# flynn-nrg/izpi

Hardware: AMD Instinct MI355X
Metric: Msamples/sec (pixels x spp) at 1024x1024/512spp (higher is better)
Workload: dtype f64

## Files before the change

### include/izpi_gpu.h

```cpp
#ifndef IZPI_GPU_H
#define IZPI_GPU_H
#include <stddef.h>
#include <stdint.h>
#include "izpi_types.h"

#ifdef __cplusplus
extern "C" {
#endif

typedef struct izpi_ctx izpi_ctx;

typedef struct izpi_scene_desc {
  uint32_t abi_version;
  uint32_t num_nodes;
  uint32_t num_prims;
  uint32_t num_tris, num_spheres, num_lights, num_materials, num_textures;
  uint32_t num_spd;
  uint32_t flags;
  uint64_t num_texels;
  const izpi_bvh4_node* nodes;
  const uint32_t* prim_ref;
  const double* tri_v0;
  const double* tri_v1;
  const double* tri_v2;
  const double* tri_e1;
  const double* tri_e2;
  const double* tri_normal;
  const double* tri_tangent;
  const double* tri_bitangent;
  const double* tri_uv;
  const double* tri_area;
  const uint32_t* tri_mat;
  const double* sph_center0;
  const double* sph_center1;
  const double* sph_time;
  const double* sph_radius;
  const uint32_t* sph_mat;
  const uint32_t* light_ref;
  const izpi_material* materials;
  const izpi_texture* textures;
  const double* texels;
  const double* spd_wavelengths;
  const double* spd_values;
  izpi_camera camera;
} izpi_scene_desc;

enum {
  IZPI_SCENE_QUANTIZED_BVH = 1
};

enum {
  IZPI_SAMPLER_NORMAL = 1,
  IZPI_SAMPLER_COLOUR = 2,
  IZPI_SAMPLER_WIREFRAME = 3,
  IZPI_SAMPLER_ALBEDO = 4,
  IZPI_SAMPLER_SPECTRAL = 5
};
enum {
  IZPI_OUT_CANVAS = 0,
  IZPI_OUT_PACKED = 1
};

typedef struct izpi_render_tuning {
  uint32_t slots;
  uint32_t chunk_units;
  uint32_t rec_dense;
  uint32_t pool_div;
  uint32_t trace_chunk;
  uint32_t refill_min;
  uint32_t prim_weight;
  uint32_t flags;
  uint64_t tail_paths;
  uint32_t peer_timeout_ms;
  uint32_t pad_tuning;
} izpi_render_tuning;
enum {
  IZPI_TUNE_NO_DIST = 1,
  IZPI_TUNE_GENERAL_TRACE = 2,
  IZPI_TUNE_NO_LEAF_SHORTCUT = 4,
  IZPI_TUNE_SCALAR_SLAB = 8,
  IZPI_TUNE_NO_TAIL = 16,
  IZPI_TUNE_PASS_LOG = 32,
  IZPI_TUNE_NO_LDS_BVH = 64,
  IZPI_TUNE_NO_RAY_LDS = 128,
  IZPI_TUNE_NO_PRIM_LDS = 256,
  IZPI_TUNE_NO_PLACE_PICK = 512,
  IZPI_TUNE_NO_QNODES = 1024,
  IZPI_TUNE_NO_SHADE_STAGE = 2048,
  IZPI_TUNE_WIDE_ADDR = 4096
};

typedef struct izpi_render_req {
  uint32_t width, height;
  uint32_t spp;
  uint32_t max_depth;
  uint32_t sampler;
  uint32_t out_layout;
  uint32_t num_tiles;
  uint32_t num_bg_spd;
  const uint32_t* tiles;
  const double* bg_spd_wavelengths;
  const double* bg_spd_values;
  double background[3];
  uint64_t seed;
  uint32_t post;
  uint32_t abi_version;
  double exposure;
  const izpi_render_tuning* tuning;
  uint32_t accumulation;
  uint32_t pad_req;
  double ink[3];
} izpi_render_req;

enum { IZPI_ACC_RECURSIVE = 0, IZPI_ACC_FORWARD = 1 };

enum { IZPI_POST_NONE = 0, IZPI_POST_SPECTRAL = 1,
       IZPI_POST_GAMMA_CLAMP = 2 };

enum { IZPI_FILTER_GAMMA = 1,
       IZPI_FILTER_CLAMP = 2   };
#define IZPI_MAX_FILTERS 8

typedef struct izpi_render_stats {
  uint64_t rays;
  uint64_t node_visits;
  uint64_t tri_tests;
  uint64_t sph_tests;
  uint64_t light_tri_tests;
  uint64_t light_sph_tests;
  uint64_t samples;
  double kernel_ms;
  double shade_ms;
  double total_ms;
  uint32_t launches;
  uint32_t pad;
  uint64_t node_steps, prim_steps, leaf_shortcuts;
  double tail_ms;
  uint64_t tail_node_visits, tail_tri_tests, tail_sph_tests;
  uint64_t parks;
  uint64_t workspace_bytes, scene_bytes;
  uint32_t slots, rec_dense, pool_blocks, chunk_spp;
  double alloc_ms;
} izpi_render_stats;

typedef struct izpi_hit {
  double t, u, v;
  double p[3];
  double normal[3];
  uint32_t prim_ref;
  uint32_t hit;
} izpi_hit;

int izpi_gpu_open(int device, izpi_ctx** out);
int izpi_gpu_close(izpi_ctx* ctx);
const char* izpi_gpu_last_error(izpi_ctx* ctx);

int izpi_gpu_upload_scene(izpi_ctx* ctx, const izpi_scene_desc* scene);

int izpi_gpu_render(izpi_ctx* ctx, const izpi_render_req* req, double* out_host, izpi_render_stats* stats);

int izpi_gpu_prepare(izpi_ctx* ctx, const izpi_render_req* req);

int izpi_gpu_render_device(izpi_ctx* ctx, const izpi_render_req* req, double* out_dev, izpi_render_stats* stats);

int izpi_gpu_unpack_tiles(izpi_ctx* ctx, const izpi_render_req* req, const double* packed_dev, double* canvas_dev);

int izpi_gpu_spectral_post(izpi_ctx* ctx, const double* xyz_dev, double* rgba_dev, uint32_t width, uint32_t height,
                           double exposure);

int izpi_gpu_postprocess(izpi_ctx* ctx, double* canvas_dev, uint32_t width, uint32_t height, const uint32_t* filters,
                         const double* params, uint32_t num_filters);

typedef struct izpi_denoise_params {
  uint32_t iterations;
  uint32_t flags;
  double sigma_colour, sigma_normal, sigma_albedo;
} izpi_denoise_params;
#define IZPI_DENOISE_MAX_ITERATIONS 8
#define IZPI_DENOISE_DEFAULT_ITERATIONS 5
#define IZPI_DENOISE_DEFAULT_SIGMA_COLOUR 1.0
#define IZPI_DENOISE_DEFAULT_SIGMA_NORMAL 0.5
#define IZPI_DENOISE_DEFAULT_SIGMA_ALBEDO 0.5
int izpi_gpu_denoise_device(izpi_ctx* ctx, const double* colour_dev, const double* normal_dev, const double* albedo_dev,
                            double* out_dev, uint32_t width, uint32_t height, const izpi_denoise_params* p,
                            double* device_ms);
int izpi_gpu_denoise(izpi_ctx* ctx, const double* colour, const double* normal, const double* albedo, double* out,
                     uint32_t width, uint32_t height, const izpi_denoise_params* p, double* device_ms);

enum { IZPI_BVH_LBVH = 0,
       IZPI_BVH_PLOC = 1,
       IZPI_BVH_SAH = 0x100 };
int izpi_gpu_build_bvh4(izpi_ctx* ctx, const double* boxes, uint32_t n, uint32_t leaf_max, uint32_t method,
                        izpi_bvh4_node* nodes, uint32_t max_nodes, uint32_t* num_nodes, uint32_t* order, double* build_ms);

typedef struct izpi_multi izpi_multi;
int izpi_gpu_multi_open(const int* devices, uint32_t num_devices, izpi_multi** out);
int izpi_gpu_multi_close(izpi_multi* m);
const char* izpi_gpu_multi_last_error(izpi_multi* m);
uint32_t izpi_gpu_multi_size(izpi_multi* m);
izpi_ctx* izpi_gpu_multi_context(izpi_multi* m, uint32_t i);
int izpi_gpu_multi_upload_scene(izpi_multi* m, const izpi_scene_desc* scene);
int izpi_gpu_multi_prepare(izpi_multi* m, const izpi_render_req* req);
int izpi_gpu_multi_render(izpi_multi* m, const izpi_render_req* req, double* out_host, izpi_render_stats* stats);

#define IZPI_COMM_ID_BYTES 128
int izpi_gpu_comm_id(uint8_t* id );
int izpi_gpu_comm_init(izpi_ctx* ctx, uint32_t nranks, uint32_t rank, const uint8_t* id );
int izpi_gpu_render_rank(izpi_ctx* ctx, const izpi_render_req* req, double* out_dev, izpi_render_stats* stats);

int izpi_gpu_progress(izpi_ctx* ctx, uint64_t* samples_done, uint64_t* samples_total);
int izpi_gpu_multi_progress(izpi_multi* m, uint64_t* samples_done, uint64_t* samples_total);

enum { IZPI_SNAP_CANVAS = 0, IZPI_SNAP_DISPLAY = 1 };
int izpi_gpu_progressive_begin(izpi_ctx* ctx, const izpi_render_req* req, uint32_t step_spp);
int izpi_gpu_progressive_step(izpi_ctx* ctx, uint32_t spp, izpi_render_stats* stats);
int izpi_gpu_progressive_snapshot(izpi_ctx* ctx, uint32_t form, double* out_host);
int izpi_gpu_progressive_snapshot_device(izpi_ctx* ctx, uint32_t form, double* out_dev);
int izpi_gpu_progressive_end(izpi_ctx* ctx);
int izpi_gpu_multi_progressive_begin(izpi_multi* m, const izpi_render_req* req, uint32_t step_spp);
int izpi_gpu_multi_progressive_step(izpi_multi* m, uint32_t spp, izpi_render_stats* stats);
int izpi_gpu_multi_progressive_snapshot(izpi_multi* m, uint32_t form, double* out_host);
int izpi_gpu_multi_progressive_end(izpi_multi* m);

enum { IZPI_PROG_NOISE = 1 };
enum { IZPI_SNAP_NOISE = 2 };
typedef struct izpi_noise_params {
  double threshold, floor, tolerated;
  uint32_t min_spp;
  uint32_t flags;
} izpi_noise_params;
#define IZPI_NOISE_DEFAULT_THRESHOLD 0.25
#define IZPI_NOISE_DEFAULT_FLOOR 0.01
#define IZPI_NOISE_DEFAULT_TOLERATED 0.05
#define IZPI_NOISE_DEFAULT_MIN_SPP 8
typedef struct izpi_noise_stats {
  uint64_t pixels, nonfinite, above;
  double max_error, sum_error, device_ms;
  uint32_t done, converged;
} izpi_noise_stats;
int izpi_gpu_progressive_begin_ex(izpi_ctx* ctx, const izpi_render_req* req, uint32_t step_spp, uint32_t flags);
int izpi_gpu_progressive_noise(izpi_ctx* ctx, const izpi_noise_params* p, izpi_noise_stats* out);
int izpi_gpu_progressive_converge(izpi_ctx* ctx, const izpi_noise_params* p, izpi_render_stats* stats,
// ... 17 lines not shown
```

### izpi_amd/_native.py

```python
import ctypes as C
from pathlib import Path

ROOT = Path(__file__).resolve().parents[1]
LIB_PATH = ROOT / "izpi_amd" / "_lib" / "libizpi_gpu.so"

c_double_p = C.POINTER(C.c_double)
c_uint32_p = C.POINTER(C.c_uint32)
c_float_p = C.POINTER(C.c_float)

COMM_ID_BYTES = 128
IZPI_OK, IZPI_ERR_INVALID, IZPI_ERR_HIP, IZPI_ERR_NO_SCENE, IZPI_ERR_UNSUPPORTED, IZPI_ERR_DEVICE, IZPI_ERR_PEER = range(7)
IZPI_ABI_VERSION = 4
ACC_RECURSIVE, ACC_FORWARD = 0, 1
SCENE_QUANTIZED_BVH = 1
PRIM_TRIANGLE, PRIM_SPHERE = 0, 1
TEX_CONSTANT, TEX_IMAGE, TEX_SPECTRAL_GAUSSIAN, TEX_SPECTRAL_TABULATED, TEX_SPECTRAL_IMAGE = 1, 3, 5, 7, 9
MAT_DIELECTRIC, MAT_DIFFUSE_LIGHT, MAT_ISOTROPIC, MAT_LAMBERT, MAT_METAL, MAT_PBR = 1, 2, 3, 4, 5, 6
MATF_BEER_LAMBERT = 1
SAMPLER_NORMAL, SAMPLER_COLOUR, SAMPLER_WIREFRAME, SAMPLER_ALBEDO, SAMPLER_SPECTRAL = 1, 2, 3, 4, 5
OUT_CANVAS, OUT_PACKED = 0, 1
POST_NONE, POST_SPECTRAL, POST_GAMMA_CLAMP = 0, 1, 2
SNAP_CANVAS, SNAP_DISPLAY, SNAP_NOISE = 0, 1, 2
PROG_NOISE = 1
NOISE_DEFAULT_THRESHOLD, NOISE_DEFAULT_FLOOR, NOISE_DEFAULT_TOLERATED, NOISE_DEFAULT_MIN_SPP = 0.25, 0.01, 0.05, 8
FILTER_GAMMA, FILTER_CLAMP = 1, 2
MAX_FILTERS = 8
HOST_SKIP_BVH = 1
BVH_LBVH, BVH_PLOC = 0, 1
BVH_SAH = 0x100
BVH_PLOC_SAH = BVH_PLOC | BVH_SAH
DISPLACE_PER_TRIANGLE, DISPLACE_MESH = 0, 1
DISPLACE_MAX_LEVELS = 16
DENOISE_MAX_ITERATIONS = 8
DENOISE_DEFAULT_ITERATIONS = 5
DENOISE_DEFAULT_SIGMA_COLOUR, DENOISE_DEFAULT_SIGMA_NORMAL, DENOISE_DEFAULT_SIGMA_ALBEDO = 1.0, 0.5, 0.5


def prim_ref(kind, idx):
    return (kind << 31) | idx


class BVH4Node(C.Structure):
    _fields_ = [("min_x", C.c_float * 4), ("min_y", C.c_float * 4), ("min_z", C.c_float * 4),
                ("max_x", C.c_float * 4), ("max_y", C.c_float * 4), ("max_z", C.c_float * 4),
                ("child", C.c_int32 * 4), ("prim_count", C.c_int32 * 4)]


class Texture(C.Structure):
    _fields_ = [("kind", C.c_uint32), ("width", C.c_uint32), ("height", C.c_uint32),
                ("spd_offset", C.c_uint32), ("spd_count", C.c_uint32), ("pad0", C.c_uint32),
                ("texel_offset", C.c_uint64), ("value", C.c_double * 3),
                ("peak", C.c_double), ("center", C.c_double), ("width_nm", C.c_double)]


class Material(C.Structure):
    _fields_ = [("kind", C.c_uint32), ("albedo_tex", C.c_int32), ("spectral_tex", C.c_int32),
                ("normal_tex", C.c_int32), ("roughness_tex", C.c_int32), ("metalness_tex", C.c_int32),
                ("absorb_tex", C.c_int32), ("flags", C.c_uint32), ("ref_idx", C.c_double),
                ("fuzz", C.c_double), ("rgb", C.c_double * 3), ("pad1", C.c_double)]


class Camera(C.Structure):
    _fields_ = [("origin", C.c_double * 3), ("lower_left", C.c_double * 3), ("horizontal", C.c_double * 3),
                ("vertical", C.c_double * 3), ("u", C.c_double * 3), ("v", C.c_double * 3),
                ("lens_radius", C.c_double), ("time0", C.c_double), ("time1", C.c_double), ("exposure", C.c_double)]


class SceneDesc(C.Structure):
    _fields_ = [("abi_version", C.c_uint32), ("num_nodes", C.c_uint32), ("num_prims", C.c_uint32),
                ("num_tris", C.c_uint32), ("num_spheres", C.c_uint32), ("num_lights", C.c_uint32),
                ("num_materials", C.c_uint32), ("num_textures", C.c_uint32), ("num_spd", C.c_uint32),
                ("flags", C.c_uint32), ("num_texels", C.c_uint64),
                ("nodes", C.POINTER(BVH4Node)), ("prim_ref", c_uint32_p),
                ("tri_v0", c_double_p), ("tri_v1", c_double_p), ("tri_v2", c_double_p),
                ("tri_e1", c_double_p), ("tri_e2", c_double_p), ("tri_normal", c_double_p),
                ("tri_tangent", c_double_p), ("tri_bitangent", c_double_p), ("tri_uv", c_double_p),
                ("tri_area", c_double_p), ("tri_mat", c_uint32_p),
                ("sph_center0", c_double_p), ("sph_center1", c_double_p), ("sph_time", c_double_p),
                ("sph_radius", c_double_p), ("sph_mat", c_uint32_p),
                ("light_ref", c_uint32_p), ("materials", C.POINTER(Material)), ("textures", C.POINTER(Texture)),
                ("texels", c_double_p), ("spd_wavelengths", c_double_p), ("spd_values", c_double_p),
                ("camera", Camera)]


class RenderTuning(C.Structure):
    _fields_ = [("slots", C.c_uint32), ("chunk_units", C.c_uint32), ("rec_dense", C.c_uint32),
                ("pool_div", C.c_uint32), ("trace_chunk", C.c_uint32), ("refill_min", C.c_uint32),
                ("prim_weight", C.c_uint32), ("flags", C.c_uint32), ("tail_paths", C.c_uint64),
                ("peer_timeout_ms", C.c_uint32), ("pad_tuning", C.c_uint32)]


TUNE_NO_DIST, TUNE_GENERAL_TRACE, TUNE_NO_LEAF_SHORTCUT, TUNE_SCALAR_SLAB, TUNE_NO_TAIL, TUNE_PASS_LOG = 1, 2, 4, 8, 16, 32
TUNE_NO_LDS_BVH = 64
TUNE_NO_RAY_LDS = 128
TUNE_NO_PRIM_LDS = 256
TUNE_NO_QNODES = 1024
TUNE_NO_SHADE_STAGE = 2048
TUNE_WIDE_ADDR = 4096


def tuning(**kw):
    t = RenderTuning()
    for k, v in kw.items():
        if k == "flags" and not isinstance(v, int):
            v = sum(v)
        setattr(t, k, v)
    return t


class RenderReq(C.Structure):
    _fields_ = [("width", C.c_uint32), ("height", C.c_uint32), ("spp", C.c_uint32), ("max_depth", C.c_uint32),
                ("sampler", C.c_uint32), ("out_layout", C.c_uint32), ("num_tiles", C.c_uint32),
                ("num_bg_spd", C.c_uint32), ("tiles", c_uint32_p), ("bg_spd_wavelengths", c_double_p),
                ("bg_spd_values", c_double_p), ("background", C.c_double * 3), ("seed", C.c_uint64),
                ("post", C.c_uint32), ("abi_version", C.c_uint32), ("exposure", C.c_double),
                ("tuning", C.POINTER(RenderTuning)), ("accumulation", C.c_uint32), ("pad_req", C.c_uint32),
                ("ink", C.c_double * 3)]


class RenderStats(C.Structure):
    _fields_ = [("rays", C.c_uint64), ("node_visits", C.c_uint64), ("tri_tests", C.c_uint64),
                ("sph_tests", C.c_uint64), ("light_tri_tests", C.c_uint64), ("light_sph_tests", C.c_uint64),
                ("samples", C.c_uint64), ("kernel_ms", C.c_double), ("shade_ms", C.c_double),
                ("total_ms", C.c_double), ("launches", C.c_uint32), ("pad", C.c_uint32),
                ("node_steps", C.c_uint64), ("prim_steps", C.c_uint64), ("leaf_shortcuts", C.c_uint64),
                ("tail_ms", C.c_double), ("tail_node_visits", C.c_uint64), ("tail_tri_tests", C.c_uint64),
                ("tail_sph_tests", C.c_uint64), ("parks", C.c_uint64), ("workspace_bytes", C.c_uint64),
                ("scene_bytes", C.c_uint64), ("slots", C.c_uint32), ("rec_dense", C.c_uint32),
                ("pool_blocks", C.c_uint32), ("chunk_spp", C.c_uint32), ("alloc_ms", C.c_double)]

    def as_dict(self):
        return {k: getattr(self, k) for k, _ in self._fields_ if k != "pad"}


class DenoiseParams(C.Structure):
    _fields_ = [("iterations", C.c_uint32), ("flags", C.c_uint32), ("sigma_colour", C.c_double),
                ("sigma_normal", C.c_double), ("sigma_albedo", C.c_double)]


def denoise_params(iterations=DENOISE_DEFAULT_ITERATIONS, sigma_colour=DENOISE_DEFAULT_SIGMA_COLOUR,
                   sigma_normal=DENOISE_DEFAULT_SIGMA_NORMAL, sigma_albedo=DENOISE_DEFAULT_SIGMA_ALBEDO):
    return DenoiseParams(int(iterations), 0, float(sigma_colour), float(sigma_normal), float(sigma_albedo))


class NoiseParams(C.Structure):
    _fields_ = [("threshold", C.c_double), ("floor", C.c_double), ("tolerated", C.c_double),
                ("min_spp", C.c_uint32), ("flags", C.c_uint32)]


def noise_params(threshold=NOISE_DEFAULT_THRESHOLD, floor=NOISE_DEFAULT_FLOOR, tolerated=NOISE_DEFAULT_TOLERATED,
                 min_spp=NOISE_DEFAULT_MIN_SPP):
    return NoiseParams(float(threshold), float(floor), float(tolerated), int(min_spp), 0)


class NoiseStats(C.Structure):
    _fields_ = [("pixels", C.c_uint64), ("nonfinite", C.c_uint64), ("above", C.c_uint64),
                ("max_error", C.c_double), ("sum_error", C.c_double), ("device_ms", C.c_double),
                ("done", C.c_uint32), ("converged", C.c_uint32)]

    def as_dict(self):
        return {k: getattr(self, k) for k, _ in self._fields_}


class Hit(C.Structure):
    _fields_ = [("t", C.c_double), ("u", C.c_double), ("v", C.c_double), ("p", C.c_double * 3),
                ("normal", C.c_double * 3), ("prim_ref", C.c_uint32), ("hit", C.c_uint32)]


class TriIn(C.Structure):
    _fields_ = [("v0", C.c_double * 3), ("v1", C.c_double * 3), ("v2", C.c_double * 3),
                ("uv", C.c_double * 6), ("material", C.c_uint32), ("pad", C.c_uint32)]


class SphereIn(C.Structure):
    _fields_ = [("center", C.c_double * 3), ("radius", C.c_double), ("material", C.c_uint32), ("pad", C.c_uint32)]


class CameraIn(C.Structure):
    _fields_ = [("look_from", C.c_double * 3), ("look_at", C.c_double * 3), ("vup", C.c_double * 3),
                ("vfov", C.c_double), ("aspect", C.c_double), ("aperture", C.c_double), ("focus_dist", C.c_double),
                ("time0", C.c_double), ("time1", C.c_double), ("exposure", C.c_double)]


class SceneInput(C.Structure):
    _fields_ = [("num_tris", C.c_uint32), ("num_spheres", C.c_uint32), ("num_materials", C.c_uint32),
                ("num_textures", C.c_uint32), ("num_spd", C.c_uint32), ("pad0", C.c_uint32),
                ("num_texels", C.c_uint64), ("tris", C.c_void_p), ("spheres", C.c_void_p),
                ("materials", C.POINTER(Material)), ("textures", C.POINTER(Texture)), ("texels", c_double_p),
                ("spd_wavelengths", c_double_p), ("spd_values", c_double_p), ("camera", CameraIn),
                ("aspect_override", C.c_double), ("bvh_seed", C.c_uint64)]


COLOUR_RGB, COLOUR_SPECTRAL = 1, 2
OBJ_IGNORE_NORMALS, OBJ_IGNORE_MATERIALS, OBJ_IGNORE_TEXTURES = 1, 2, 4
OBJ_FACE_POLYGON = 1


class ProtoInfo(C.Structure):
    _fields_ = [("colour_representation", C.c_uint32), ("stream_triangles", C.c_uint32),
                ("total_triangles", C.c_uint64), ("num_triangles", C.c_uint32), ("num_streamed_triangles", C.c_uint32),
                ("num_spheres", C.c_uint32), ("num_materials", C.c_uint32), ("num_image_textures", C.c_uint32),
                ("num_displacement_maps", C.c_uint32), ("num_background", C.c_uint32), ("pad", C.c_uint32),
                ("name", C.c_char_p), ("version", C.c_char_p), ("warnings", C.c_char_p)]


class ObjInfo(C.Structure):
    _fields_ = [("has_normals", C.c_uint32), ("has_uv", C.c_uint32), ("ignore_materials", C.c_uint32),
                ("ignore_normals", C.c_uint32), ("ignore_textures", C.c_uint32), ("num_groups", C.c_uint32),
                ("num_materials", C.c_uint32), ("pad", C.c_uint32), ("num_vertices", C.c_uint64),
                ("num_normals", C.c_uint64), ("num_uvs", C.c_uint64), ("centre", C.c_double * 3),
                ("object_name", C.c_char_p)]


class ObjGroup(C.Structure):
    _fields_ = [("name", C.c_char_p), ("material", C.c_char_p), ("face_type", C.c_uint32), ("is_null", C.c_uint32),
                ("num_faces", C.c_uint64), ("num_face_vertices", C.c_uint64)]


class ObjMaterial(C.Structure):
    _fields_ = [("name", C.c_char_p), ("kd", C.c_double * 3), ("ka", C.c_double * 3), ("ks", C.c_double * 3),
                ("num_kd", C.c_uint32), ("num_ka", C.c_uint32), ("num_ks", C.c_uint32), ("pad", C.c_uint32),
                ("ns", C.c_double), ("ni", C.c_double), ("d", C.c_double), ("sharpness", C.c_int64),
                ("illum", C.c_int64)]


ABI_STRUCTS = [BVH4Node, Texture, Material, Camera, SceneDesc, RenderReq, RenderStats, Hit, TriIn, SphereIn, CameraIn,
               SceneInput, ProtoInfo, ObjInfo, ObjGroup, ObjMaterial, RenderTuning, DenoiseParams, NoiseParams, NoiseStats]

EXPORTS = [
    "izpi_gpu_open", "izpi_gpu_close", "izpi_gpu_prepare", "izpi_gpu_multi_prepare", "izpi_gpu_last_error", "izpi_gpu_upload_scene", "izpi_gpu_render",
    "izpi_gpu_render_device", "izpi_gpu_unpack_tiles", "izpi_gpu_output_bytes", "izpi_gpu_trace",
    "izpi_gpu_ray_aabb4", "izpi_gpu_gomath", "izpi_gpu_spectral_post", "izpi_gpu_postprocess",
    "izpi_gpu_build_bvh4", "izpi_gpu_multi_open", "izpi_gpu_multi_close", "izpi_gpu_multi_last_error",
    "izpi_gpu_multi_size", "izpi_gpu_multi_context", "izpi_gpu_multi_upload_scene", "izpi_gpu_multi_render",
    "izpi_gpu_comm_id", "izpi_gpu_comm_init", "izpi_gpu_render_rank", "izpi_gpu_debug_fault", "izpi_gpu_debug_realloc", "izpi_gpu_progress", "izpi_gpu_multi_progress", "izpi_host_build_scene_ex", "izpi_host_scene_prim_boxes", "izpi_host_scene_set_bvh", "izpi_host_scene_set_flags",
    "izpi_host_build_scene", "izpi_host_scene_desc", "izpi_host_scene_stack_bound", "izpi_host_scene_build_ms",
    "izpi_host_scene_free", "izpi_host_last_error", "izpi_host_tiles", "izpi_host_share_units", "izpi_host_share_tiles", "izpi_host_share_block", "izpi_host_assemble_shares", "izpi_host_bvh_leaf_max", "izpi_host_gomath", "izpi_abi_struct_size",
    "izpi_scene_parse_text", "izpi_scene_parse_binary", "izpi_scene_serialize", "izpi_scene_info", "izpi_scene_image_file",
    "izpi_scene_set_image", "izpi_scene_add_triangles", "izpi_scene_background", "izpi_scene_to_input",
    "izpi_scene_material_name", "izpi_scene_free", "izpi_light_source", "izpi_light_source_name",
    "izpi_obj_parse", "izpi_obj_info_get", "izpi_obj_copy_vertices", "izpi_obj_group_get", "izpi_obj_copy_faces",
    "izpi_obj_material_get", "izpi_obj_translate", "izpi_obj_scale", "izpi_obj_rotate",
    "izpi_obj_group_to_triangles", "izpi_obj_free",
    "izpi_gpu_displace", "izpi_host_displace", "izpi_scene_displacement_file", "izpi_scene_set_displacement_map",
    "izpi_scene_set_displacer",
    "izpi_gpu_progressive_begin", "izpi_gpu_progressive_step", "izpi_gpu_progressive_snapshot",
    "izpi_gpu_progressive_snapshot_device", "izpi_gpu_progressive_end",
    "izpi_gpu_multi_progressive_begin", "izpi_gpu_multi_progressive_step", "izpi_gpu_multi_progressive_snapshot",
    "izpi_gpu_multi_progressive_end",
    "izpi_gpu_denoise_device", "izpi_gpu_denoise", "izpi_host_denoise",
    "izpi_gpu_progressive_begin_ex", "izpi_gpu_progressive_noise", "izpi_gpu_progressive_converge",
# ... 144 lines not shown
```

### izpi_amd/csrc/izpi_dev.h

```cpp
#pragma once
#include <hip/hip_runtime.h>
#include <stdint.h>
#include "../../include/izpi_gpu.h"
#include "gomath.h"
#include "scene_records.h"

#define IZPI_DEV __device__ __forceinline__

namespace izd {

struct DevScene {
  const GInner* inner;
  const GInnerQ* innerq;
  const GLeaf* leaves;
  const GPrim* prims;
  const GShade* shade;
  const GTriTex* tritex;
  const GLight* lights;
  const izpi_material* materials;
  const izpi_texture* textures;
  const double4* mat_const;
  const MatTex* mat_tex;
  const double* texels;
  const double* spd_wl;
  const double* spd_val;
  int32_t root;
  uint32_t num_lights;
  uint32_t nan_free_bounds;
  uint32_t leaf_shortcut;
  uint32_t tri_only;
  uint32_t no_pathlen;
  uint32_t num_inner;
  uint32_t num_prims;
  izpi_camera cam;
  uint32_t lds_bytes;
  uint32_t time_free;
  uint32_t quantized;
  uint32_t addr32;
#ifdef IZPI_SHADOW
  const GInner* sh_inner;
  const GLeaf* sh_leaves;
  const GPrim* sh_prims;
#endif
};

struct RenderParams {
  uint32_t width, height, spp, max_depth;
  uint32_t chunk_spp;
  uint32_t s0;
  uint32_t num_pixels;
  uint32_t tile_w, tile_h;
  uint32_t total_units;
  uint32_t lanes;
  uint32_t num_bg_spd;
  const uint32_t* tiles;
  const double* bg_wl;
  const double* bg_val;
  double background[3];
  uint64_t seed;
  double* out;
  double* recs;
  uint32_t* head;
  unsigned long long* counters;
  uint32_t* error;
};

struct Lcg {
  uint32_t s;
  IZPI_DEV double next() {
    s = 1664525u * s + 1013904223u;
    return (double)s / 4294967296.0;
  }
};
IZPI_DEV uint64_t splitmix64(uint64_t x) {
  uint64_t z = x + 0x9E3779B97F4A7C15ull;
  z = (z ^ (z >> 30)) * 0xBF58476D1CE4E5B9ull;
  z = (z ^ (z >> 27)) * 0x94D049BB133111EBull;
  return z ^ (z >> 31);
}
#define IZPI_CAMERA_STREAM_SALT 0xD6E8FEB86659FD93ull

IZPI_DEV int64_t go_int(double x) {
  if (x != x || x >= 9223372036854775808.0 || x < -9223372036854775808.0) return INT64_MIN;
  return (int64_t)x;
}

struct V3 { double x, y, z; };
IZPI_DEV V3 mk(double x, double y, double z) { V3 r; r.x = x; r.y = y; r.z = z; return r; }
IZPI_DEV V3 ld3(const double* p) { return mk(p[0], p[1], p[2]); }
IZPI_DEV V3 add(V3 a, V3 b) { return mk(a.x + b.x, a.y + b.y, a.z + b.z); }
IZPI_DEV V3 sub(V3 a, V3 b) { return mk(a.x - b.x, a.y - b.y, a.z - b.z); }
IZPI_DEV V3 mul(V3 a, V3 b) { return mk(a.x * b.x, a.y * b.y, a.z * b.z); }
IZPI_DEV V3 smul(V3 a, double t) { return mk(a.x * t, a.y * t, a.z * t); }
IZPI_DEV bool sdiv_plain(double x) {
  return ((uint32_t)(__double2hiint(x) >> 20) & 0x7FFu) - (1023u - 300u) <= 600u;
}
IZPI_DEV V3 sdiv(V3 a, double t) {
  const int px = (int)sdiv_plain(a.x) | (int)(a.x == 0.0), py = (int)sdiv_plain(a.y) | (int)(a.y == 0.0),
            pz = (int)sdiv_plain(a.z) | (int)(a.z == 0.0);
  const bool plain = ((int)sdiv_plain(t) & px & py & pz) != 0;
  if (plain) {
    double r = __builtin_amdgcn_rcp(t);
    double e = __builtin_fma(-t, r, 1.0);
    r = __builtin_fma(r, e, r);
    e = __builtin_fma(-t, r, 1.0);
    r = __builtin_fma(r, e, r);
    auto q1 = [&](double n) {
      const double q = n * r;
      const double res = __builtin_fma(-t, q, n);
      return __builtin_amdgcn_div_fixup(__builtin_amdgcn_div_fmas(res, r, q, false), t, n);
    };
    return mk(q1(a.x), q1(a.y), q1(a.z));
  }
  return mk(a.x / t, a.y / t, a.z / t);
}
IZPI_DEV double dot(V3 a, V3 b) { return (a.x * b.x) + (a.y * b.y) + (a.z * b.z); }
IZPI_DEV V3 cross(V3 a, V3 b) { return mk((a.y * b.z) - (a.z * b.y), -((a.x * b.z) - (a.z * b.x)), (a.x * b.y) - (a.y * b.x)); }
IZPI_DEV double sqlen(V3 a) { return (a.x * a.x) + (a.y * a.y) + (a.z * a.z); }
IZPI_DEV double length(V3 a) { return gm::sqrt(sqlen(a)); }
IZPI_DEV V3 unit(V3 a) { return sdiv(a, length(a)); }
IZPI_DEV V3 lerp(V3 a, V3 b, double t) {
  return mk((1 - t) * a.x + t * b.x, (1 - t) * a.y + t * b.y, (1 - t) * a.z + t * b.z);
}
IZPI_DEV bool bad(double x) { return x != x || gm::is_inf(x, 0); }
IZPI_DEV V3 denan(V3 v) { return mk(bad(v.x) ? 0.0 : v.x, bad(v.y) ? 0.0 : v.y, bad(v.z) ? 0.0 : v.z); }

struct Onb {
  V3 u, v, w;
  IZPI_DEV void build(V3 n) {
    w = unit(n);
    V3 a = gm::abs(w.x) > 0.9 ? mk(0, 1, 0) : mk(1, 0, 0);
    v = unit(cross(w, a));
    u = cross(w, v);
  }
  IZPI_DEV V3 local(V3 a) const { return add(add(smul(u, a.x), smul(v, a.y)), smul(w, a.z)); }
};

IZPI_DEV V3 random_cosine_direction(Lcg& r) {
  double r1 = r.next();
  double r2 = r.next();
  double z = gm::sqrt(1 - r2);
  double phi = 6.283185307179586 * r1;
  double sp, cp;
  gm::sincos_nonneg(phi, &sp, &cp);
  double x = cp * 2 * gm::sqrt(r2);
  double y = sp * 2 * gm::sqrt(r2);
  return mk(x, y, z);
}
IZPI_DEV V3 random_to_sphere(double radius, double dist2, Lcg& r) {
  double r1 = r.next();
  double r2 = r.next();
  double z = 1 + r2 * (gm::sqrt(1 - radius * radius / dist2) - 1);
  double phi = 6.283185307179586 * r1;
  double sp, cp;
  gm::sincos_nonneg(phi, &sp, &cp);
  double x = cp * gm::sqrt(1 - z * z);
  double y = sp * gm::sqrt(1 - z * z);
  return mk(x, y, z);
}
IZPI_DEV V3 random_in_unit_sphere(Lcg& r) {
  for (;;) {
    double x = r.next(), y = r.next(), z = r.next();
    V3 p = sub(smul(mk(x, y, z), 2.0), mk(1.0, 1.0, 1.0));
    if (sqlen(p) < 1.0) return p;
  }
}

IZPI_DEV float max32(float a, float b) { return a > b ? a : b; }
IZPI_DEV float min32(float a, float b) { return a < b ? a : b; }
IZPI_DEV bool slab(float mnx, float mny, float mnz, float mxx, float mxy, float mxz, float ox, float oy, float oz,
                   float ix, float iy, float iz, float tmax) {
  float t0x = (mnx - ox) * ix, t1x = (mxx - ox) * ix;
  if (t0x > t1x) { float t = t0x; t0x = t1x; t1x = t; }
  float t0y = (mny - oy) * iy, t1y = (mxy - oy) * iy;
  if (t0y > t1y) { float t = t0y; t0y = t1y; t1y = t; }
  float t0z = (mnz - oz) * iz, t1z = (mxz - oz) * iz;
  if (t0z > t1z) { float t = t0z; t0z = t1z; t1z = t; }
  float tn = max32(max32(t0x, t0y), t0z);
  float tf = min32(min32(t1x, t1y), t1z);
  return tn <= tf && tf >= 0 && tn <= tmax;
}

typedef float f32x2 __attribute__((ext_vector_type(2)));
IZPI_DEV void slab4_fast(float4 mnx, float4 mny, float4 mnz, float4 mxx, float4 mxy, float4 mxz, float ox, float oy,
                         float oz, float ix, float iy, float iz, float tmax, uint64_t (&h)[4]) {
  const f32x2 o_x = {ox, ox}, o_y = {oy, oy}, o_z = {oz, oz};
  const f32x2 i_x = {ix, ix}, i_y = {iy, iy}, i_z = {iz, iz};
  const f32x2 a0x = (f32x2{mnx.x, mnx.y} - o_x) * i_x, a1x = (f32x2{mnx.z, mnx.w} - o_x) * i_x;
  const f32x2 b0x = (f32x2{mxx.x, mxx.y} - o_x) * i_x, b1x = (f32x2{mxx.z, mxx.w} - o_x) * i_x;
  const f32x2 a0y = (f32x2{mny.x, mny.y} - o_y) * i_y, a1y = (f32x2{mny.z, mny.w} - o_y) * i_y;
  const f32x2 b0y = (f32x2{mxy.x, mxy.y} - o_y) * i_y, b1y = (f32x2{mxy.z, mxy.w} - o_y) * i_y;
// ... 87 lines not shown
```

### izpi_amd/csrc/izpi_gpu.hip

```cpp
#include "izpi_kern.h"
#include "noise.h"
#include "scene_pack.h"

#include <array>

using izpi_internal::Double4;
using izpi_internal::pack_scene;
using izpi_internal::PackedScene;
using izpi_internal::trace_addr32;
using izpi_internal::trace_layout;
using izpi_internal::TraceLayout;
using izpi_internal::PlanCache;
using izpi_internal::PlanInput;
using izpi_internal::SideLayout;
using izpi_internal::WorkspacePlan;

__global__ void __launch_bounds__(256) k_spectral_post(const double* in, double* out, uint32_t W, uint32_t H,
                                                       double exposure) {
  __shared__ double ys[18][18];
  const int tx = threadIdx.x & 15, ty = threadIdx.x >> 4;
  const int x0 = blockIdx.x * 16, y0 = blockIdx.y * 16;
  for (int i = threadIdx.x; i < 18 * 18; i += 256) {
    const int hx = x0 + (i % 18) - 1, hy = y0 + (i / 18) - 1;
    ys[i / 18][i % 18] = (hx >= 0 && hx < (int)W && hy >= 0 && hy < (int)H) ? in[((size_t)hy * W + hx) * 4 + 1] : 0.0;
// ... 418 lines not shown

int allocate(izpi_ctx* ctx, const izpi_render_req* req, const RequestShape& rs, const WorkspacePlan& plan, const Tracer& tr,
             const RenderCall& call) {
  const auto bufs = ctx_buffers(ctx);
  const size_t bytes[RENDER_BUFS] = {plan.samples_bytes, plan.recs_bytes, plan.pool_bytes, plan.ring_bytes,
                                     plan.running_bytes, plan.state_bytes, tr.spill_bytes};
  int rc = IZPI_OK;
  if (rs.preview) {
    if ((rc = session_keeps_sums(ctx, call, ctx->running_cap < plan.running_bytes))) return rc;
    for (size_t k = 0; k < RENDER_BUFS && !rc; k++) rc = grow(ctx, bufs[k].p, bufs[k].cap, bytes[k]);
  } else {
    bool fresh = false;
    rc = grow_render_buffers(ctx, bufs.data(), bytes, &fresh);
    if (!rc && (rc = session_keeps_sums(ctx, call, fresh))) return rc;
  }
  if (!rc) rc = grow(ctx, (void**)&ctx->d_tiles, &ctx->tiles_cap, rs.tiles.size() * sizeof(uint32_t));
  if (!rc && !rs.preview) {
    if (req->num_bg_spd && (!req->bg_spd_wavelengths || !req->bg_spd_values)) { ctx->err = "num_bg_spd without the SPD arrays"; return IZPI_ERR_INVALID; }
    rc = grow(ctx, (void**)&ctx->d_bg, &ctx->bg_cap, (2 * (size_t)req->num_bg_spd + 1) * sizeof(double));
  }
  if (!rc) rc = grow(ctx, (void**)&ctx->d_cpart, &ctx->cpart_cap, (size_t)cpart_rows(ctx) * CNT_N * sizeof(unsigned long long));
  if (!rc && !rs.preview && !rs.fwd) rc = grow(ctx, (void**)&ctx->d_finq, &ctx->finq_cap, (size_t)ctx->num_cus * CPART_BLOCKS_PER_CU * FINQ_WORDS * FINQ_CAP * sizeof(unsigned long long));
  if (rc) ctx->plans[rs.preview].valid = false;
  return rc;
}

int touch_workspace(izpi_ctx* ctx, const WorkspacePlan& plan, const RenderCall& call, double alloc_ms) {
  hipStream_t st = ctx->stream;
  HIP_TRY(hipMemsetAsync(ctx->d_state, 0, plan.state_bytes, st));
  HIP_TRY(hipMemsetAsync(ctx->d_samples, 0, plan.samples_bytes, st));
  if (plan.recs_bytes) HIP_TRY(hipMemsetAsync(ctx->d_recs, 0, plan.recs_bytes, st));
  if (call.range.keep) {
    HIP_TRY(hipMemsetAsync(ctx->d_running, 0, plan.running_bytes, st));
    HIP_TRY(hipMemsetAsync(ctx->d_counters, 0, CNT_N * sizeof(unsigned long long), st));
  }
  HIP_TRY(hipStreamSynchronize(st));
  ctx->last = izpi_render_stats{};
  ctx->last.workspace_bytes = workspace_bytes(ctx);
  ctx->last.slots = plan.slots; ctx->last.chunk_spp = plan.chunk; ctx->last.alloc_ms = alloc_ms;
  return IZPI_OK;
}

int begin_frame(izpi_ctx* ctx, const izpi_render_req* req, const RequestShape& rs, const WorkspacePlan& plan, const RenderCall& call,
                size_t nbg) {
  hipStream_t st = ctx->stream;
  HIP_TRY(hipMemcpyAsync(ctx->d_tiles, rs.tiles.data(), rs.tiles.size() * sizeof(uint32_t), hipMemcpyHostToDevice, st));
  if (nbg) {
    HIP_TRY(hipMemcpyAsync(ctx->d_bg, req->bg_spd_wavelengths, nbg * sizeof(double), hipMemcpyHostToDevice, st));
    HIP_TRY(hipMemcpyAsync(ctx->d_bg + nbg, req->bg_spd_values, nbg * sizeof(double), hipMemcpyHostToDevice, st));
  }
  if (!call.range.keep) {
    HIP_TRY(hipMemsetAsync(ctx->d_running, 0, plan.running_bytes, st));
    HIP_TRY(hipMemsetAsync(ctx->d_counters, 0, CNT_N * sizeof(unsigned long long), st));
  }
  HIP_TRY(hipMemsetAsync(ctx->d_cpart, 0, (size_t)cpart_rows(ctx) * CNT_N * sizeof(unsigned long long), st));
  HIP_TRY(hipMemsetAsync(ctx->d_misc, 0, 8 * MISC_STRIDE * sizeof(uint32_t), st));
  return IZPI_OK;
}

ShadeParams shade_params(izpi_ctx* ctx, const izpi_render_req* req, const RequestShape& rs, const WorkspacePlan& plan) {
  ShadeParams sp{};
  sp.width = req->width; sp.height = req->height; sp.tile_w = rs.tw; sp.tile_h = rs.th; sp.slots = plan.slots;
  sp.max_depth = rs.preview ? 1 : req->max_depth;
  sp.tiles = ctx->d_tiles; sp.seed = req->seed; sp.out = ctx->d_samples;
  sp.background[0] = req->background[0]; sp.background[1] = req->background[1]; sp.background[2] = req->background[2];
  sp.counters = ctx->d_counters; sp.cpart = ctx->d_cpart; sp.error = misc(ctx, 1);
  return sp;
}
void path_shade_params(izpi_ctx* ctx, const izpi_render_req* req, const DevScene& sc, const RequestShape& rs,
                       const WorkspacePlan& plan, size_t nbg, ShadeParams& sp) {
  sp.num_bg_spd = (uint32_t)nbg;
  sp.bg_sorted = nbg >= 2;
  for (size_t i = 1; i < nbg; i++)
    if (!(req->bg_spd_wavelengths[i - 1] <= req->bg_spd_wavelengths[i])) sp.bg_sorted = 0;
  sp.bg_wl = ctx->d_bg; sp.bg_val = ctx->d_bg + nbg;
  sp.rec_dense = plan.rec_dense; sp.rec_pool = plan.rec_pool; sp.pool_shift = plan.pool_shift;
  sp.recs = rs.fwd ? nullptr : ctx->d_recs; sp.mat_const = sc.mat_const; sp.head = misc(ctx, 0);
  sp.num_mc = ctx->num_materials; sp.num_tex = ctx->num_textures; sp.num_spd = ctx->num_spd;
  sp.pool = plan.rec_pool ? ctx->d_pool : nullptr; sp.pool_ring = plan.rec_pool ? ctx->d_ring : nullptr;
  sp.pool_ctr = plan.rec_pool ? ctx->d_pool_ctr : nullptr;
  sp.finq = ctx->d_finq;
}
void stage_tables(const izpi_ctx* ctx, const izpi_render_req* req, const izpi_render_tuning& tu, const RequestShape& rs,
                  const WorkspacePlan& plan, size_t nbg, DevScene& sc, ShadeParams& sp) {
  sp.staged = ctx->num_materials <= MC_LDS && ctx->num_materials <= MAT_LDS && sc.num_lights <= LT_LDS &&
              ctx->num_textures <= TEX_LDS && ctx->num_spd <= SPD_LDS && nbg <= BG_LDS;
  sp.prims_staged = sc.num_prims <= PR_LDS && !(tu.flags & IZPI_TUNE_NO_PRIM_LDS);
  if (sp.staged && (req->sampler == IZPI_SAMPLER_SPECTRAL || ctx->num_spd)) sp.staged = 2;
  if (rs.fwd && req->sampler == IZPI_SAMPLER_COLOUR && ctx->matset == 0 && sp.staged == 1 && !plan.rec_pool && !plan.time &&
      !plan.cold && !(tu.flags & IZPI_TUNE_NO_SHADE_STAGE))
    sp.prims_staged = 0;
  sc.lds_bytes = sp.prims_staged ? lds_off::END : sp.staged == 2 ? lds_off::SPECTRAL_END : sp.staged ? lds_off::COLOUR_END : 0;
  if (tu.flags & IZPI_TUNE_PASS_LOG)
    fprintf(stderr, "IZPI_SHADE_TABLES tables=%u prims=%u lds_bytes=%u\n", sp.staged, sp.prims_staged, sc.lds_bytes);
}
WaveParams wave_params(izpi_ctx* ctx, const WorkspacePlan& plan, const ShadeParams& sp) {
  WaveParams wp{};
  wp.in = bind_side(ctx->d_state, plan, plan.side[0]); wp.out = bind_side(ctx->d_state, plan, plan.side[1]);
  wp.trace_next = misc(ctx, 2); wp.slots = plan.slots;
  wp.read_kind = !ctx->sc.no_pathlen ? 1u : 0u;
  wp.hit_uv = plan.uv ? 1u : 0u;
  wp.pool_ctr = sp.pool_ctr;
  wp.cpart = ctx->d_cpart;
  return wp;
}
PreviewParams preview_params(izpi_ctx* ctx, const izpi_render_req* req, const WorkspacePlan& plan) {
  PreviewParams pp{};
  pp.buf = bind_side(ctx->d_state, plan, plan.side[0]);
  pp.tminmax = plan.tminmax ? (double2*)(ctx->d_state + plan.side[0].tminmax) : nullptr;
  pp.slots = plan.slots;
  pp.verts = ctx->d_triverts;
  if (req->abi_version >= 4)
    for (int k = 0; k < 3; k++) pp.ink[k] = req->ink[k];
  return pp;
}
AccumParams accum_params(izpi_ctx* ctx, const izpi_render_req* req, const RequestShape& rs, double* out_dev) {
  AccumParams ap{};
  ap.num_pixels = rs.num_pixels; ap.spp = req->spp; ap.width = req->width; ap.height = req->height;
  ap.tile_w = rs.tw; ap.tile_h = rs.th; ap.out_layout = req->out_layout;
  ap.sampler = rs.preview ? (uint32_t)IZPI_SAMPLER_COLOUR : req->sampler;
  ap.tiles = ctx->d_tiles; ap.samples = ctx->d_samples; ap.running = ctx->d_running; ap.out = out_dev;
  return ap;
}

int guard_status(izpi_ctx* ctx, uint32_t guard) {
  if (!guard) return IZPI_OK;
  ctx->err = guard & 1u   ? "device guard: traversal stack overflow"
             : guard & 2u ? "device guard: unknown material kind"
                            : "device guard: no overflow record block in k_tail";
  return IZPI_ERR_DEVICE;
}

int render_body(izpi_ctx* ctx, const izpi_render_req* req, const RenderCall& call, double* out_dev) {
  const auto t_body0 = std::chrono::steady_clock::now();
  auto host_ms = [&t_body0]() { return std::chrono::duration<double, std::milli>(std::chrono::steady_clock::now() - t_body0).count(); };
  RequestShape rs;
  int rc = check_request(ctx, req, &rs);
  if (rc) return rc;
  const SampleRange& sr = call.range;
  const uint32_t num_pixels = rs.num_pixels;
  if (sr.keep) {
    izpi_ctx::Session& ss = ctx->session;
    ss.run_tiles = rs.tiles; ss.tile_w = rs.tw; ss.tile_h = rs.th; ss.num_pixels = num_pixels;
  }
  const izpi_render_tuning& tu = tuning_of(req);
  const bool pass_log = (tu.flags & IZPI_TUNE_PASS_LOG) != 0;
  DevScene sc = ctx->sc;
  if (tu.flags & IZPI_TUNE_NO_LEAF_SHORTCUT) sc.leaf_shortcut = 0;
  if (tu.flags & IZPI_TUNE_SCALAR_SLAB) sc.nan_free_bounds = 0;
  Tracer tr;
  const double t_tiles = host_ms();
  if ((rc = make_tracer(ctx, tu, !ctx->sc.tri_only || ctx->any_uv, &tr))) return rc;
  if (pass_log)
    fprintf(stderr, "IZPI_TRACE_INSTANCE dist=%d tri=%d lds_bvh=%d ray_lds=%d q=%d\nIZPI_TRACE_ADDR a32=%d ring=%d\n", (int)tr.p2, (int)tr.tri,
            (int)tr.lds_bvh, (int)tr.ray_lds, (int)tr.qnodes, (int)(tr.a32 && !tr.lds_bvh), trace_ring(tr));
  const double t_tracer = host_ms();
  PlanCache& cache = ctx->plans[rs.preview];
  PlanInput in = plan_input(ctx, req, rs, tu, call.size_spp);
  const bool reuse = cache.find(in) != nullptr;
  if (!reuse) in.avail = available_bytes(ctx);
  const double t_meminfo = host_ms();
  if (!reuse) cache.store(in, plan_workspace(in));
  const WorkspacePlan& plan = cache.plan;
  const double t_sized = host_ms();
  const auto t_alloc0 = std::chrono::steady_clock::now();
  if ((rc = allocate(ctx, req, rs, plan, tr, call))) return rc;
  const double alloc_ms = std::chrono::duration<double, std::milli>(std::chrono::steady_clock::now() - t_alloc0).count();
  if (call.prepare_only) return touch_workspace(ctx, plan, call, alloc_ms);
  hipStream_t st = ctx->stream;
  if (pass_log) HIP_TRY(hipEventRecord(ctx->evb[0], st));
  const size_t nbg = rs.preview ? 0 : req->num_bg_spd;
  if ((rc = begin_frame(ctx, req, rs, plan, call, nbg))) return rc;
  ShadeParams sp = shade_params(ctx, req, rs, plan);
  AccumParams ap = accum_params(ctx, req, rs, out_dev);
  if (!rs.preview) {
    path_shade_params(ctx, req, sc, rs, plan, nbg, sp);
    stage_tables(ctx, req, tu, rs, plan, nbg, sc, sp);
  }

  const RunInput run{num_pixels, plan.chunk, plan.pool_blocks, sr};
  RunTimes times;
  float total_ms = 0;
  const double t_launch = host_ms();
  HIP_TRY(hipEventRecord(ctx->ev0, st));
  if (pass_log) {
    HIP_TRY(hipEventSynchronize(ctx->ev0));
    float prep = 0;
    HIP_TRY(hipEventElapsedTime(&prep, ctx->evb[0], ctx->ev0));
    fprintf(stderr, "IZPI_T ev0_synced %.3f prep_gpu_ms %.3f body_start %.3f\n", diag_clock_ms(), prep,
            diag_clock_ms() - host_ms());
  }
  if (rs.preview) {
    const PreviewParams pp = preview_params(ctx, req, plan);
    rc = run_preview(ctx, req, sc, tr, sp, pp, ap, run, &times);
  } else {
    WaveParams wp = wave_params(ctx, plan, sp);
    const ShadeKernels* k = ctx->kernels[req->sampler == IZPI_SAMPLER_SPECTRAL][rs.fwd];
    if (!k || (!rs.fwd && k->rec_doubles != plan.D)) {
      ctx->err = "the shading instance and the workspace plan disagree on the record stride";
      return IZPI_ERR_INVALID;
    }
    rc = run_wavefront(ctx, req, sc, tr, *k, sp, wp, ap, run, &times);
  }
  if (rc) return rc;
  hipLaunchKernelGGL(k_cpart_reduce, dim3(CNT_N), dim3(256), 0, st, ctx->d_cpart, cpart_rows(ctx), ctx->d_counters);
  HIP_TRY(hipGetLastError());
  HIP_TRY(hipEventRecord(ctx->ev1, st));
  if (!sr.keep && (rc = apply_post(ctx, req, out_dev))) return rc;
  const double t_issued = host_ms();
  HIP_TRY(hipEventSynchronize(ctx->ev1));
  if (pass_log)
    fprintf(stderr, "IZPI_HOST tiles %.3f tracer %.3f meminfo %.3f sized %.3f allocated %.3f launched %.3f issued %.3f done %.3f ms\n",
            t_tiles, t_tracer, t_meminfo, t_sized, t_sized + alloc_ms, t_launch, t_issued, host_ms());
  HIP_TRY(hipEventElapsedTime(&total_ms, ctx->ev0, ctx->ev1));
  unsigned long long cnt[CNT_N];
  uint32_t guard = 0;
  HIP_TRY(hipMemcpy(cnt, ctx->d_counters, sizeof(cnt), hipMemcpyDeviceToHost));
  HIP_TRY(hipMemcpy(&guard, misc(ctx, 1), sizeof(guard), hipMemcpyDeviceToHost));
  izpi_render_stats& s = ctx->last;
  memset(&s, 0, sizeof(s));
  s.rays = cnt[CNT_RAYS]; s.node_visits = cnt[CNT_NODES]; s.tri_tests = cnt[CNT_TRI]; s.sph_tests = cnt[CNT_SPH];
  s.light_tri_tests = cnt[CNT_LTRI]; s.light_sph_tests = cnt[CNT_LSPH];
  s.samples = (uint64_t)num_pixels * sr.end;
  s.kernel_ms = times.trace_ms; s.shade_ms = times.shade_ms; s.total_ms = total_ms; s.launches = times.launches; s.tail_ms = times.tail_ms;
  s.node_steps = cnt[CNT_NSTEP]; s.prim_steps = cnt[CNT_PSTEP]; s.leaf_shortcuts = cnt[CNT_SHORT];
  s.tail_node_visits = cnt[CNT_TAIL_NODES]; s.tail_tri_tests = cnt[CNT_TAIL_TRI]; s.tail_sph_tests = cnt[CNT_TAIL_SPH];
  s.parks = cnt[CNT_PARK];
  s.workspace_bytes = workspace_bytes(ctx);
  s.scene_bytes = ctx->scene_bytes;
  s.slots = plan.slots; s.rec_dense = rs.fwd ? 0 : plan.rec_dense; s.pool_blocks = plan.pool_blocks; s.chunk_spp = plan.chunk;
  s.alloc_ms = alloc_ms;
  if (!sr.keep && plan.rec_pool && s.parks * 64 > s.rays && plan.pool_blocks < plan.slots) ctx->pool_grow++;
#ifdef IZPI_SHADE_CLOCKS
  fprintf(stderr, "IZPI_SHADE_CLOCKS item %llu refill %llu push %llu mat %llu finish %llu mix %llu lpdf %llu entry %llu tex %llu "
          "res_barrier1 %llu res_atomics %llu res_barrier2 %llu (wave cycles; res_atomics: thread 0 only)\n",
          cnt[CNT_SCLK_ITEM], cnt[CNT_SCLK_REFILL], cnt[CNT_SCLK_PUSH], cnt[CNT_SCLK_MAT], cnt[CNT_SCLK_FIN],
          cnt[CNT_SCLK_MIX], cnt[CNT_SCLK_LPDF], cnt[CNT_SCLK_ENTRY], cnt[CNT_SCLK_TEX], cnt[CNT_SCLK_RB1],
          cnt[CNT_SCLK_RATOM], cnt[CNT_SCLK_RB2]);
#endif
#ifdef IZPI_SHADOW
  fprintf(stderr, "IZPI_SHADOW spill_stores %llu spill_loads %llu (entries)\n", cnt[CNT_CLK_REFILL], cnt[CNT_CLK_NODE]);
#endif
#ifdef IZPI_TRACE_ICOUNT
  fprintf(stderr, "IZPI_TRACE_ICOUNT {\"iterations\": %llu, \"idle\": %llu, \"dequeue\": %llu, \"refill\": %llu, \"prim\": %llu, \"node_fast\": %llu, "
          "\"node_twin\": %llu, \"spill\": %llu, \"readback\": %llu, \"pop\": %llu, \"finish\": %llu, \"waves\": %llu}\n",
          cnt[CNT_IC_ITER], cnt[CNT_IC_IDLE], cnt[CNT_IC_DEQUEUE], cnt[CNT_IC_REFILL], cnt[CNT_PSTEP], cnt[CNT_NSTEP] - cnt[CNT_IC_TWIN], cnt[CNT_IC_TWIN],
          cnt[CNT_IC_SPILL], cnt[CNT_IC_READBACK], cnt[CNT_IC_POP], cnt[CNT_IC_FINISH], cnt[CNT_IC_WAVES]);
#endif
#ifdef IZPI_TRACE_CLOCKS
  fprintf(stderr, "IZPI_TRACE_CLOCKS refill %llu node %llu prim %llu advance %llu (wave cycles)\n", cnt[CNT_CLK_REFILL],
          cnt[CNT_CLK_NODE], cnt[CNT_CLK_PRIM], cnt[CNT_CLK_ADV]);
#endif
  return guard_status(ctx, guard);
}

int render_impl(izpi_ctx* ctx, const izpi_render_req* req, const RenderCall& call, double* out_dev) {
  if (session_open(ctx)) return IZPI_ERR_INVALID;
  ctx->prog_done.store(0, std::memory_order_relaxed);
  ctx->prog_total.store(0, std::memory_order_relaxed);
  const int rc = render_body(ctx, req, call, out_dev);
  ctx->prog_done.store(ctx->prog_total.load(std::memory_order_relaxed), std::memory_order_relaxed);
  return rc;
}

struct Shares {
  std::vector<uint32_t> all;
  uint32_t n = 1;
  uint32_t tw = 0, th = 0;
  size_t block = 0;
  std::vector<uint32_t> mine(uint32_t r) const {
    std::vector<uint32_t> t(all.size());
    t.resize(4 * (size_t)izpi_host_share_tiles(all.data(), (uint32_t)(all.size() / 4), r, n, t.data()));
    return t;
  }
};

size_t share_block(size_t ntiles, uint32_t tw, uint32_t th, uint32_t n) { return ((ntiles + n - 1) / n) * (size_t)tw * th * 4; }

int make_shares(izpi_ctx* ctx, const izpi_render_req* req, uint32_t n, Shares& sh) {
  if (!req || req->width == 0 || req->height == 0) { ctx->err = "invalid render request"; return IZPI_ERR_INVALID; }
  if (req->out_layout != IZPI_OUT_CANVAS) { ctx->err = "multi-GPU renders produce a canvas (IZPI_OUT_CANVAS)"; return IZPI_ERR_INVALID; }
  std::vector<uint32_t> tiles;
  int rc = request_tiles(ctx, req, tiles);
  if (rc) return rc;
  sh.all.resize(4 * tiles.size());
  sh.all.resize(4 * (size_t)izpi_host_share_units(tiles.data(), (uint32_t)(tiles.size() / 4), n, sh.all.data()));
  if (!validate_tiles(req, sh.all.data(), (uint32_t)(sh.all.size() / 4), &sh.tw, &sh.th)) {
    ctx->err = "tiles must be non-empty, in bounds and equal-sized";
    return IZPI_ERR_INVALID;
  }
  sh.n = n;
  sh.block = share_block(sh.all.size() / 4, sh.tw, sh.th, n);
  return IZPI_OK;
}

int share_buffers(izpi_ctx* ctx, const Shares& sh, bool root, size_t canvas_bytes = 0) {
  int rc = grow(ctx, (void**)&ctx->d_share, &ctx->share_cap, sh.block * sizeof(double));
  if (!rc && root) rc = grow(ctx, (void**)&ctx->d_gather, &ctx->gather_cap, (size_t)sh.n * sh.block * sizeof(double));
  if (!rc && root && canvas_bytes) rc = grow(ctx, (void**)&ctx->d_out, &ctx->out_cap, canvas_bytes);
  return rc;
}

int render_share(izpi_ctx* ctx, const izpi_render_req* req, const Shares& sh, uint32_t r, bool prepare_only = false) {
  const std::vector<uint32_t> mine = sh.mine(r);
  memset(&ctx->last, 0, sizeof(ctx->last));
  if (mine.empty()) return IZPI_OK;
  izpi_render_req q = request_copy(req);
  q.num_tiles = (uint32_t)(mine.size() / 4);
  q.tiles = mine.data();
  q.out_layout = IZPI_OUT_PACKED;
  q.post = IZPI_POST_NONE;
  return render_impl(ctx, &q, one_shot(&q, prepare_only), prepare_only ? nullptr : ctx->d_share);
}

int assemble(izpi_ctx* ctx, const izpi_render_req* req, const Shares& sh, double* canvas_dev) {
  izpi_ctx* root = ctx;
  hipStream_t st = root->stream;
  for (uint32_t r = 0; r < sh.n; r++) {
    const std::vector<uint32_t> t = sh.mine(r);
    if (t.empty()) continue;
    int rc = grow(root, (void**)&root->d_utiles, &root->utiles_cap, sh.all.size() * sizeof(uint32_t));
    if (rc) return rc;
    HIP_TRY(hipMemcpyAsync(root->d_utiles, t.data(), t.size() * sizeof(uint32_t), hipMemcpyHostToDevice, st));
    const uint32_t np = (uint32_t)(t.size() / 4) * sh.tw * sh.th;
    hipLaunchKernelGGL(k_unpack, dim3((np + 255) / 256), dim3(256), 0, st, root->d_utiles, np, sh.tw, sh.th, req->width,
                       req->height, root->d_gather + (size_t)r * sh.block, canvas_dev);
    HIP_TRY(hipGetLastError());
    HIP_TRY(hipStreamSynchronize(st));
  }
  int rc = apply_post(root, req, canvas_dev);
  if (rc) return rc;
  HIP_TRY(hipStreamSynchronize(st));
  return IZPI_OK;
}

int session_copy_request(izpi_ctx::Session& ss, const izpi_render_req* req, std::string& err) {
  ss = izpi_ctx::Session{};
  ss.req = request_copy(req);
  ss.tuning = tuning_of(req);
  ss.req.tuning = req->tuning ? &ss.tuning : nullptr;
  if (ss.req.num_tiles) {
    if (!ss.req.tiles) { err = "num_tiles without tiles"; return IZPI_ERR_INVALID; }
    ss.tiles.assign(ss.req.tiles, ss.req.tiles + 4 * (size_t)ss.req.num_tiles);
    ss.req.tiles = ss.tiles.data();
  }
  if (ss.req.num_bg_spd) {
    if (!ss.req.bg_spd_wavelengths || !ss.req.bg_spd_values) { err = "num_bg_spd without the SPD arrays"; return IZPI_ERR_INVALID; }
    ss.bg_wl.assign(ss.req.bg_spd_wavelengths, ss.req.bg_spd_wavelengths + ss.req.num_bg_spd);
    ss.bg_val.assign(ss.req.bg_spd_values, ss.req.bg_spd_values + ss.req.num_bg_spd);
    ss.req.bg_spd_wavelengths = ss.bg_wl.data();
    ss.req.bg_spd_values = ss.bg_val.data();
  }
  return IZPI_OK;
}

void session_drop(izpi_ctx* ctx) {
  ctx->session = izpi_ctx::Session{};
  ctx->prog_done.store(0, std::memory_order_relaxed);
  ctx->prog_total.store(0, std::memory_order_relaxed);
}

int session_zero_moments(izpi_ctx* ctx) {
  izpi_ctx::Session& ss = ctx->session;
  const size_t bytes = (size_t)ss.num_pixels * 3 * sizeof(double);
  const int rc = grow(ctx, (void**)&ctx->d_moments, &ctx->moments_cap, bytes);
  if (rc) return rc;
  HIP_TRY(hipMemsetAsync(ctx->d_moments, 0, bytes, ctx->stream));
  HIP_TRY(hipStreamSynchronize(ctx->stream));
  ss.noise = true;
  return IZPI_OK;
}

int session_begin(izpi_ctx* ctx, const izpi_render_req* req, uint32_t step_spp, uint32_t flags = 0) {
  if (ctx->session.open) { ctx->err = "a progressive session is already open"; return IZPI_ERR_INVALID; }
  if (!req || step_spp == 0) { ctx->err = "progressive_begin: a request and step_spp >= 1"; return IZPI_ERR_INVALID; }
  if (flags & ~(uint32_t)IZPI_PROG_NOISE) { ctx->err = "progressive_begin: unknown flags"; return IZPI_ERR_INVALID; }
  izpi_ctx::Session& ss = ctx->session;
  int rc = session_copy_request(ss, req, ctx->err);
  if (!rc) {
    ss.step_spp = std::min(step_spp, std::max(1u, ss.req.spp));
    rc = render_body(ctx, &ss.req, RenderCall{SampleRange{0, 0, true}, ss.step_spp, true}, nullptr);
  }
  if (!rc && (flags & IZPI_PROG_NOISE)) rc = session_zero_moments(ctx);
  if (rc) {
    const std::string why = ctx->err;
    session_drop(ctx);
    ctx->err = why;
    return rc;
  }
  ss.cum = izpi_render_stats{};
  ss.open = true;
  ctx->prog_done.store(0, std::memory_order_relaxed);
  ctx->prog_total.store((uint64_t)ss.num_pixels * ss.req.spp, std::memory_order_relaxed);
  return IZPI_OK;
}

int session_usable(izpi_ctx* ctx) {
  if (!ctx->session.open) { ctx->err = "no progressive session is open"; return IZPI_ERR_INVALID; }
  if (ctx->session.broken) { ctx->err = "the session's last step failed: end it"; return IZPI_ERR_INVALID; }
  return IZPI_OK;
// ... 86 lines not shown
  return IZPI_OK;
}

template <class Step, class Noise, class Done>
int converge_loop(const izpi_noise_params* params, uint32_t cap, Step step, Noise noise, Done done, izpi_noise_stats* out) {
  const izpi_noise_params p = params ? *params : nz::defaults();
  izpi_noise_stats last{};
  int rc = IZPI_OK;
  while (!rc && done() < cap) {
    if ((rc = step())) break;
    if (done() < std::max(2u, p.min_spp)) continue;
    if ((rc = noise(&p, &last))) break;
    if (last.converged) break;
  }
  if (out) *out = last;
  return rc;
}

int session_snapshot(izpi_ctx* ctx, uint32_t form, double* out_dev) {
  int rc = session_usable(ctx);
  if (rc) return rc;
  const izpi_ctx::Session& ss = ctx->session;
  if (form != IZPI_SNAP_CANVAS && form != IZPI_SNAP_DISPLAY && form != IZPI_SNAP_NOISE) { ctx->err = "unknown snapshot form"; return IZPI_ERR_INVALID; }
  if (ss.done == 0) { ctx->err = "snapshot before the session's first sample"; return IZPI_ERR_INVALID; }
  if (form == IZPI_SNAP_NOISE && (rc = session_has_noise(ctx))) return rc;
  if (!out_dev) { ctx->err = "null output"; return IZPI_ERR_INVALID; }
  hipStream_t st = ctx->stream;
  if ((rc = session_tiles(ctx))) return rc;
  if (form == IZPI_SNAP_NOISE) {
    NoiseParams np = noise_params(ctx);
    np.out = out_dev;
    launch_noise_resolve(st, np);
    HIP_TRY(hipGetLastError());
    HIP_TRY(hipStreamSynchronize(st));
    return IZPI_OK;
  }
  ResolveParams rp{};
  rp.num_pixels = ss.num_pixels; rp.done = ss.done; rp.width = ss.req.width; rp.height = ss.req.height;
  rp.tile_w = ss.tile_w; rp.tile_h = ss.tile_h; rp.sampler = ss.req.sampler; rp.out_layout = ss.req.out_layout;
  rp.form = form; rp.exposure = ss.req.exposure;
  rp.tiles = ctx->d_tiles; rp.running = ctx->d_running; rp.out = out_dev;
  launch_resolve(st, rp);
  HIP_TRY(hipGetLastError());
  if (form == IZPI_SNAP_CANVAS && (rc = apply_post(ctx, &ss.req, out_dev))) return rc;
  HIP_TRY(hipStreamSynchronize(st));
  return IZPI_OK;
}

}

struct izpi_multi {
  std::vector<izpi_ctx*> ctx;
  std::string err;
  bool prog_open = false;
  izpi_ctx::Session session;
  Shares shares;
};

namespace {
int multi_shares(izpi_multi* m, const izpi_render_req* req, Shares& sh) {
  izpi_ctx* root = m->ctx[0];
  int rc = make_shares(root, req, (uint32_t)m->ctx.size(), sh);
  if (!rc && hipSetDevice(root->device) != hipSuccess) { root->err = "hipSetDevice"; rc = IZPI_ERR_HIP; }
  if (!rc) rc = share_buffers(root, sh, true, (size_t)req->width * req->height * 4 * sizeof(double));
  if (rc) m->err = root->err;
  return rc;
}

template <class F>
int on_every_device(izpi_multi* m, F fn) {
  const uint32_t G = (uint32_t)m->ctx.size();
  std::vector<int> rcs(G, IZPI_OK);
  std::vector<std::thread> th;
  for (uint32_t i = 0; i < G; i++) {
    th.emplace_back([&, i]() {
      izpi_ctx* c = m->ctx[i];
      if (hipSetDevice(c->device) != hipSuccess) { c->err = "hipSetDevice"; rcs[i] = IZPI_ERR_HIP; return; }
      rcs[i] = fn(i, c);
    });
  }
  for (std::thread& t : th) t.join();
  for (uint32_t i = 0; i < G; i++)
    if (rcs[i]) { m->err = "device " + std::to_string(i) + ": " + m->ctx[i]->err; return rcs[i]; }
  return IZPI_OK;
}

bool multi_lacks_noise(izpi_multi* m) {
  if (!m->session.noise) { m->err = "noise: the session was begun without IZPI_PROG_NOISE"; return true; }
  if (m->session.done < 2) { m->err = "noise: needs at least 2 samples"; return true; }
  return false;
}

bool multi_session_open(izpi_multi* m) {
  if (!m->prog_open) return false;
  m->err = "a progressive session is open";
  return true;
}

static_assert(sizeof(Double4) == sizeof(double4), "PackedScene::mat_const uploads as DevScene::mat_const");

int begin_upload(izpi_ctx* ctx, const izpi_scene_desc* d) {
  if (!ctx || !d) return IZPI_ERR_INVALID;
  if (d->abi_version < 1 || d->abi_version > IZPI_ABI_VERSION) { ctx->err = "ABI version mismatch"; return IZPI_ERR_INVALID; }
  if (session_open(ctx)) return IZPI_ERR_INVALID;
  HIP_TRY(hipSetDevice(ctx->device));
  HIP_TRY(hipStreamSynchronize(ctx->stream));
  free_scene(ctx);
  return IZPI_OK;
}

int upload_packed(izpi_ctx* ctx, const izpi_scene_desc* d, const PackedScene& ps) {
  DevScene& sc = ctx->sc;
  memset(&sc, 0, sizeof(sc));
  GInner* di; GInnerQ* dq; GLeaf* dl; GPrim* dp; GShade* dsh; GTriVerts* dtv; GTriTex* dtt; GLight* dlt;
  izpi_material* dm; Double4* dmc; MatTex* dmt; izpi_texture* dtx;
  double *dtex, *dswl, *dsv;
  {
    const TraceLayout tl = trace_layout(ps.inner.size(), ps.innerq.size(), ps.leaves.size());
    char* nb;
    UP((const char*)nullptr, tl.bytes, &nb);
    di = reinterpret_cast<GInner*>(nb);
    dq = ps.innerq.empty() ? nullptr : reinterpret_cast<GInnerQ*>(nb + tl.innerq_at);
    dl = reinterpret_cast<GLeaf*>(nb + tl.leaves_at);
    HIP_TRY(hipMemcpy(di, ps.inner.data(), ps.inner.size() * sizeof(GInner), hipMemcpyHostToDevice));
    if (dq) HIP_TRY(hipMemcpy(dq, ps.innerq.data(), ps.innerq.size() * sizeof(GInnerQ), hipMemcpyHostToDevice));
    HIP_TRY(hipMemcpy(dl, ps.leaves.data(), ps.leaves.size() * sizeof(GLeaf), hipMemcpyHostToDevice));
  }
  UP(ps.prims.data(), ps.prims.size(), &dp);
  UP(ps.shade.data(), ps.shade.size(), &dsh);
  UP(ps.triverts.data(), ps.triverts.size(), &dtv);
  UP(ps.tritex.data(), ps.tritex.size(), &dtt);
  UP(ps.lights.data(), ps.lights.size(), &dlt);
  UP(d->materials, d->num_materials, &dm);
  UP(ps.mat_const.data(), ps.mat_const.size(), &dmc);
  UP(ps.mat_tex.data(), ps.mat_tex.size(), &dmt);
  UP(ps.textures.data(), ps.textures.size(), &dtx);
  UP(ps.texels.data(), ps.texels.size(), &dtex);
  UP(d->spd_wavelengths, d->num_spd, &dswl);
  UP(d->spd_values, d->num_spd, &dsv);
#ifdef IZPI_SHADOW
  {
    GInner* si; GLeaf* sl; GPrim* sp;
    UP(ps.inner.data(), ps.inner.size(), &si);
    UP(ps.leaves.data(), ps.leaves.size(), &sl);
    UP(ps.prims.data(), ps.prims.size(), &sp);
    sc.sh_inner = si; sc.sh_leaves = sl; sc.sh_prims = sp;
  }
#endif
  sc.inner = di; sc.innerq = dq; sc.leaves = dl; sc.prims = dp; sc.shade = dsh; sc.tritex = dtt; sc.lights = dlt;
  sc.materials = dm; sc.mat_const = (const double4*)dmc; sc.mat_tex = dmt; sc.textures = dtx; sc.texels = dtex;
  sc.spd_wl = dswl; sc.spd_val = dsv;
  sc.root = ps.root; sc.num_inner = ps.num_inner; sc.num_prims = d->num_prims; sc.num_lights = d->num_lights;
  sc.quantized = ps.quantized; sc.leaf_shortcut = ps.leaf_shortcut; sc.nan_free_bounds = ps.nan_free_bounds;
  sc.tri_only = ps.tri_only; sc.time_free = ps.time_free; sc.no_pathlen = ps.no_pathlen;
  sc.addr32 = trace_addr32(ps.inner.size(), ps.innerq.size(), ps.leaves.size(), ps.prims.size());
  sc.cam = d->camera;
  ctx->d_triverts = dtv;
  ctx->mat_ok_rgb = ps.mat_ok_rgb; ctx->mat_ok_spectral = ps.mat_ok_spectral;
  ctx->basic_materials = ps.basic_materials; ctx->matset = ps.matset;
  ctx->const_albedo = ps.const_albedo; ctx->any_uv = ps.any_uv;
  ctx->pool_grow = 0;
  ctx->stack_needed = ps.stack_needed;
  ctx->num_prims = d->num_prims;
  ctx->num_textures = d->num_textures;
  ctx->num_materials = d->num_materials;
  ctx->num_spd = d->num_spd;
  ctx->have_scene = true;
  ctx->plans[0].valid = ctx->plans[1].valid = false;
  Tracer tr;
  int rc = make_tracer(ctx, kDefaultTuning, !ctx->sc.tri_only || ctx->any_uv, &tr);
  const bool const_basic = ctx->basic_materials && ctx->const_albedo;
  for (int s = 0; s < 2; s++)
    for (int f = 1; f >= 0; f--) {
      const uint32_t sampler = s ? IZPI_SAMPLER_SPECTRAL : IZPI_SAMPLER_COLOUR;
      const ShadeKernels*& k = ctx->kernels[s][f];
      k = (s ? ctx->mat_ok_spectral : ctx->mat_ok_rgb) ? shade_instance(ctx->matset, const_basic, sampler, f != 0) : nullptr;
      if (!rc && k) rc = prepare_wavefront(ctx, *k);
    }
  if (!rc) rc = prepare_preview(ctx);
  return rc;
}
}

extern "C" {

int izpi_gpu_open(int device, izpi_ctx** out) {
  if (!out) return IZPI_ERR_INVALID;
  *out = nullptr;
  int n = 0;
  hipError_t e = hipGetDeviceCount(&n);
  if (e != hipSuccess || n == 0 || device < 0 || device >= n) return IZPI_ERR_HIP;
  if (hipSetDevice(device) != hipSuccess) return IZPI_ERR_HIP;
  izpi_ctx* ctx = new izpi_ctx();
  ctx->device = device;
  hipDeviceProp_t prop;
  bool ok = hipGetDeviceProperties(&prop, device) == hipSuccess;
  ctx->num_cus = ok ? prop.multiProcessorCount : 0;
  ok = ok && hipStreamCreateWithFlags(&ctx->stream, hipStreamNonBlocking) == hipSuccess &&
       hipEventCreate(&ctx->ev0) == hipSuccess && hipEventCreate(&ctx->ev1) == hipSuccess &&
       hipEventCreate(&ctx->ev2) == hipSuccess && hipEventCreate(&ctx->ev3) == hipSuccess &&
       hipHostMalloc((void**)&ctx->h_count, 9 * MISC_STRIDE * sizeof(uint32_t), hipHostMallocDefault) == hipSuccess &&
       hipMalloc((void**)&ctx->d_misc, 8 * MISC_STRIDE * sizeof(uint32_t)) == hipSuccess &&
       hipMalloc((void**)&ctx->d_pool_ctr, POOL_SHARDS * POOL_CTR_STRIDE * sizeof(unsigned long long)) == hipSuccess &&
       hipMalloc((void**)&ctx->d_counters, CNT_N * sizeof(unsigned long long)) == hipSuccess;
  for (int i = 0; ok && i < 3 * IZPI_PASS_BATCH; i++) ok = hipEventCreate(&ctx->evb[i]) == hipSuccess;
  if (!ok) {
    izpi_gpu_close(ctx);
    return IZPI_ERR_HIP;
  }
  *out = ctx;
  return IZPI_OK;
}

int izpi_gpu_close(izpi_ctx* ctx) {
  if (!ctx) return IZPI_OK;
  (void)hipSetDevice(ctx->device);
  if (ctx->stream) (void)hipStreamSynchronize(ctx->stream);
  if (ctx->comm) (void)ncclCommDestroy(ctx->comm);
  free_scene(ctx);
  for (const CtxBuf& b : ctx_buffers(ctx)) if (*b.p) (void)hipFree(*b.p);
  void* fixed[] = {ctx->d_pool_ctr, ctx->d_misc, ctx->d_counters, ctx->d_status};
  for (void* p : fixed) if (p) (void)hipFree(p);
  if (ctx->h_count) (void)hipHostFree(ctx->h_count);
  if (ctx->stall_host) (void)hipHostFree(ctx->stall_host);
  for (int i = 0; i < 3 * IZPI_PASS_BATCH; i++) if (ctx->evb[i]) (void)hipEventDestroy(ctx->evb[i]);
  hipEvent_t evs[] = {ctx->ev0, ctx->ev1, ctx->ev2, ctx->ev3};
  for (hipEvent_t ev : evs) if (ev) (void)hipEventDestroy(ev);
  if (ctx->stream) (void)hipStreamDestroy(ctx->stream);
  delete ctx;
  return IZPI_OK;
}

const char* izpi_gpu_last_error(izpi_ctx* ctx) { return ctx ? ctx->err.c_str() : "null context"; }

int izpi_gpu_upload_scene(izpi_ctx* ctx, const izpi_scene_desc* d) {
  int rc = begin_upload(ctx, d);
  if (rc) return rc;
  PackedScene ps;
  rc = pack_scene(d, &ps, &ctx->err);
  return rc ? rc : upload_packed(ctx, d, ps);
}

uint64_t izpi_gpu_output_bytes(const izpi_render_req* req) {
  if (!req) return 0;
  if (req->out_layout == IZPI_OUT_PACKED && req->num_tiles) {
    uint64_t px = 0;
    for (uint32_t i = 0; i < req->num_tiles; i++) {
      const uint32_t* t = req->tiles + 4 * i;
      px += (uint64_t)(t[2] - t[0] + 1) * (t[3] - t[1] + 1);
    }
    return px * 4 * sizeof(double);
  }
  return (uint64_t)req->width * req->height * 4 * sizeof(double);
}

int izpi_gpu_render_device(izpi_ctx* ctx, const izpi_render_req* req, double* out_dev, izpi_render_stats* stats) {
  if (!ctx) return IZPI_ERR_INVALID;
  if (!out_dev) { ctx->err = "null output"; return IZPI_ERR_INVALID; }
  HIP_TRY(hipSetDevice(ctx->device));
  int rc = render_impl(ctx, req, one_shot(req), out_dev);
  if (stats) *stats = ctx->last;
  return rc;
}

int izpi_gpu_render(izpi_ctx* ctx, const izpi_render_req* req, double* out_host, izpi_render_stats* stats) {
  if (!ctx) return IZPI_ERR_INVALID;
  if (!out_host || !req) { ctx->err = "null argument"; return IZPI_ERR_INVALID; }
  if (session_open(ctx)) return IZPI_ERR_INVALID;
  HIP_TRY(hipSetDevice(ctx->device));
  const size_t bytes = izpi_gpu_output_bytes(req);
  int rc = grow(ctx, (void**)&ctx->d_out, &ctx->out_cap, bytes);
  if (rc) return rc;
  HIP_TRY(hipMemcpyAsync(ctx->d_out, out_host, bytes, hipMemcpyHostToDevice, ctx->stream));
  rc = render_impl(ctx, req, one_shot(req), ctx->d_out);
  if (stats) *stats = ctx->last;
  if (rc) return rc;
  HIP_TRY(hipMemcpyAsync(out_host, ctx->d_out, bytes, hipMemcpyDeviceToHost, ctx->stream));
  HIP_TRY(hipStreamSynchronize(ctx->stream));
  return IZPI_OK;
}

int izpi_gpu_prepare(izpi_ctx* ctx, const izpi_render_req* req) {
  if (!ctx) return IZPI_ERR_INVALID;
  if (!req) { ctx->err = "null argument"; return IZPI_ERR_INVALID; }
  if (session_open(ctx)) return IZPI_ERR_INVALID;
  HIP_TRY(hipSetDevice(ctx->device));
  if (ctx->comm && ctx->comm_size > 1) {
    Shares sh;
    int rc = make_shares(ctx, req, ctx->comm_size, sh);
    if (!rc) rc = share_buffers(ctx, sh, ctx->comm_rank == 0);
    return rc ? rc : render_share(ctx, req, sh, ctx->comm_rank, true);
  }
  return render_impl(ctx, req, one_shot(req, true), nullptr);
}

int izpi_gpu_progressive_begin_ex(izpi_ctx* ctx, const izpi_render_req* req, uint32_t step_spp, uint32_t flags) {
  if (!ctx) return IZPI_ERR_INVALID;
  HIP_TRY(hipSetDevice(ctx->device));
  return session_begin(ctx, req, step_spp, flags);
}

int izpi_gpu_progressive_begin(izpi_ctx* ctx, const izpi_render_req* req, uint32_t step_spp) {
  return izpi_gpu_progressive_begin_ex(ctx, req, step_spp, 0);
}

int izpi_gpu_progressive_noise(izpi_ctx* ctx, const izpi_noise_params* p, izpi_noise_stats* out) {
  if (!ctx) return IZPI_ERR_INVALID;
// ... 708 lines not shown
```

### izpi_amd/csrc/izpi_kern.h

```cpp
#pragma once
#include <hip/hip_runtime.h>
#include <stdio.h>
#include <stdlib.h>
#include <string.h>
#include <algorithm>
#include <cmath>
#include <string>
#include <vector>

#include <rccl/rccl.h>

#include <atomic>
#include <chrono>
#include <thread>

#include "../../include/izpi_host.h"
#include "../../include/izpi_gpu_debug.h"
#include "izpi_dev.h"
#include "izpi_req.h"
#include "render_plan.h"
#include "cie_tables.h"

using namespace izd;

#define HIP_TRY(expr)                                                                  \
  do {                                                                                 \
    hipError_t e_ = (expr);                                                            \
    if (e_ != hipSuccess) {                                                            \
      ctx->err = std::string(#expr) + ": " + hipGetErrorString(e_);                    \
      return IZPI_ERR_HIP;                                                             \
    }                                                                                  \
  } while (0)

static __constant__ double c_cie_wl[IZPI_CIE_N] = IZPI_CIE_WAVELENGTHS_INIT;
static __constant__ double c_cie_x[IZPI_CIE_N] = IZPI_CIE_X_INIT;
static __constant__ double c_cie_y[IZPI_CIE_N] = IZPI_CIE_Y_INIT;
static __constant__ double c_cie_z[IZPI_CIE_N] = IZPI_CIE_Z_INIT;
struct CieCum { double v[IZPI_CIE_N]; };
constexpr CieCum cie_y_running_sums() {
  CieCum c{};
  constexpr double y[IZPI_CIE_N] = IZPI_CIE_Y_INIT;
  double cur = 0.0;
  for (int i = 0; i < IZPI_CIE_N; i++) { c.v[i] = cur + y[i]; cur += y[i]; }
  return c;
}
static __constant__ CieCum c_cie_ycum = cie_y_running_sums();

namespace izpi_bvh {
int build(hipStream_t st, const double* h_boxes, uint32_t n, uint32_t leaf_max, uint32_t method,
          std::vector<izpi_bvh4_node>& nodes, std::vector<uint32_t>& order, float* ms, std::string& err);
}

#define IZPI_PASS_BATCH 8
constexpr uint32_t SHADE_THREADS = 256, SHADE_WAVES = SHADE_THREADS / 64;
constexpr uint32_t FINQ_WORDS = 5, FINQ_FLUSH = 1024, FINQ_CAP = FINQ_FLUSH + SHADE_THREADS;
constexpr int MISC_STRIDE = 64;

enum { CNT_RAYS = 0, CNT_NODES, CNT_TRI, CNT_SPH, CNT_LTRI, CNT_LSPH, CNT_NSTEP, CNT_PSTEP, CNT_SHORT,
       CNT_CLK_REFILL, CNT_CLK_NODE, CNT_CLK_PRIM, CNT_CLK_ADV, CNT_TAIL_NODES, CNT_TAIL_TRI, CNT_TAIL_SPH,
       CNT_SCLK_ITEM, CNT_SCLK_REFILL, CNT_SCLK_PUSH, CNT_PARK, CNT_SCLK_MAT, CNT_SCLK_FIN, CNT_SCLK_MIX, CNT_SCLK_LPDF,
       CNT_SCLK_ENTRY, CNT_SCLK_TEX, CNT_SCLK_RB1, CNT_SCLK_RATOM, CNT_SCLK_RB2,
       CNT_N };
#ifdef IZPI_TRACE_ICOUNT
enum { CNT_IC_ITER = CNT_CLK_REFILL, CNT_IC_DEQUEUE = CNT_CLK_NODE, CNT_IC_REFILL = CNT_CLK_PRIM, CNT_IC_TWIN = CNT_CLK_ADV,
       CNT_IC_SPILL = CNT_SCLK_ITEM, CNT_IC_READBACK = CNT_SCLK_REFILL, CNT_IC_POP = CNT_SCLK_PUSH, CNT_IC_FINISH = CNT_SCLK_MAT,
       CNT_IC_WAVES = CNT_SCLK_FIN, CNT_IC_IDLE = CNT_SCLK_MIX };
#if defined(IZPI_TRACE_CLOCKS) || defined(IZPI_SHADE_CLOCKS) || defined(IZPI_SHADOW)
#error "IZPI_TRACE_ICOUNT shares counter rows with the clock and shadow builds"
#endif
#endif

IZPI_DEV void count_add(unsigned long long* cpart, unsigned long long* counters, int k, unsigned long long v) {
  if (v == 0) return;
  if (cpart) cpart[(size_t)__builtin_amdgcn_readfirstlane(blockIdx.x * (blockDim.x >> 6) + (threadIdx.x >> 6)) * CNT_N + k] += v;
  else atomicAdd(counters + k, v);
}

template <class T>
IZPI_DEV T sld(const T* p) { return *p; }
template <class T>
IZPI_DEV void sst(T* p, const T& v) { *p = v; }

template <class T>
IZPI_DEV T lds_ld(const T* p) {
  if constexpr (sizeof(T) % 8 == 0 && alignof(T) >= 8) {
    T r;
    uint64_t* d = reinterpret_cast<uint64_t*>(&r);
    const __attribute__((address_space(3))) uint64_t* q = (const __attribute__((address_space(3))) uint64_t*)p;
#pragma unroll
    for (uint32_t i = 0; i < sizeof(T) / 8; i++) d[i] = q[i];
    return r;
  } else {
    return *(const __attribute__((address_space(3))) T*)p;
  }
}

template <bool L, class T>
IZPI_DEV T tld(const T* p) {
  if constexpr (L) return lds_ld(p);
  else return *p;
}
constexpr uint32_t MAT_LDS = 64, TEX_LDS = 64, SPD_LDS = 384, BG_LDS = 128, MT_LDS = 64, LT_LDS = 64, PR_LDS = 64;
namespace lds_off {
constexpr uint32_t al(uint64_t b) { return (uint32_t)((b + 31) & ~31ull); }
constexpr uint32_t MC = 0;
constexpr uint32_t MT = MC + al(MT_LDS * sizeof(double4));
constexpr uint32_t LT = MT + al(MT_LDS * sizeof(MatTex));
constexpr uint32_t LT2 = LT + al(LT_LDS * 16 * sizeof(double));
constexpr uint32_t MAT = LT2 + al(LT_LDS * 6 * sizeof(double));
constexpr uint32_t TEX = MAT + al(MAT_LDS * sizeof(izpi_material));
constexpr uint32_t COLOUR_END = TEX + al(TEX_LDS * sizeof(izpi_texture));
constexpr uint32_t SPD = COLOUR_END;
constexpr uint32_t SPDV = SPD + al(SPD_LDS * sizeof(double));
constexpr uint32_t CIE = SPDV + al(SPD_LDS * sizeof(double));
constexpr uint32_t BG = CIE + al(5 * IZPI_CIE_N * sizeof(double));
constexpr uint32_t BGV = BG + al(BG_LDS * sizeof(double));
constexpr uint32_t SPECTRAL_END = BGV + al(BG_LDS * sizeof(double));
constexpr uint32_t GS = SPECTRAL_END;
constexpr uint32_t TT = GS + al(PR_LDS * sizeof(GShade));
constexpr uint32_t GP = TT + al(PR_LDS * sizeof(GTriTex));
constexpr uint32_t END = GP + al(PR_LDS * sizeof(GPrim));
constexpr uint32_t STG_RAY = COLOUR_END;
constexpr uint32_t STG_THR = STG_RAY + 3 * SHADE_THREADS * 16;
constexpr uint32_t STG_PATH = STG_THR + 3 * SHADE_THREADS * 8;
constexpr uint32_t STG_KIND = STG_PATH + SHADE_THREADS * 16;
constexpr uint32_t STG_END = STG_KIND + SHADE_THREADS * 4;
constexpr uint32_t STG_BYTES = STG_END - COLOUR_END;
}
IZPI_DEV char* lds_arena() {
  extern __shared__ __attribute__((aligned(16))) char izpi_lds_arena[];
  return izpi_lds_arena;
}
IZPI_DEV izpi_material* mat_lds() { return (izpi_material*)(lds_arena() + lds_off::MAT); }
IZPI_DEV izpi_texture* tex_lds() { return (izpi_texture*)(lds_arena() + lds_off::TEX); }
IZPI_DEV double* spd_lds() { return (double*)(lds_arena() + lds_off::SPD); }
IZPI_DEV double* spdv_lds() { return (double*)(lds_arena() + lds_off::SPDV); }
IZPI_DEV double* cie_lds() { return (double*)(lds_arena() + lds_off::CIE); }
IZPI_DEV double* bg_lds() { return (double*)(lds_arena() + lds_off::BG); }
IZPI_DEV double* bgv_lds() { return (double*)(lds_arena() + lds_off::BGV); }
IZPI_DEV izpi_material mat_rec(const DevScene& sc, bool st, uint32_t m) {
  if (st) return lds_ld(mat_lds() + m);
  return sc.materials[m];
}
IZPI_DEV izpi_texture tex_rec(const DevScene& sc, bool st, int32_t id) {
  if (st) return lds_ld(tex_lds() + id);
  return sc.textures[id];
}

IZPI_DEV V3 image_rgb(const double* texels, uint64_t off, uint32_t w, uint32_t h, uint32_t fmt, double u, double v) {
  int64_t i = go_int(u * (double)w);
  int64_t j = go_int((1 - v) * ((double)h - 0.001));
  if (i < 0) i = 0;
  if (j < 0) j = 0;
  if (i > (int64_t)w - 1) i = (int64_t)w - 1;
  if (j > (int64_t)h - 1) j = (int64_t)h - 1;
  uint64_t k = (uint64_t)j * w + (uint64_t)i;
  if (fmt == TEXF_GRAY) {
    const double g = texels[off + k];
    return mk(g, g, g);
  }
  const double* px = texels + off + k * 4;
  const double2 rg = *reinterpret_cast<const double2*>(px);
  return mk(rg.x, rg.y, px[2]);
}
IZPI_DEV uint64_t image_index(uint32_t w, uint32_t h, double u, double v) {
  int64_t i = go_int(u * (double)w);
  int64_t j = go_int((1 - v) * ((double)h - 0.001));
  if (i < 0) i = 0;
  if (j < 0) j = 0;
  if (i > (int64_t)w - 1) i = (int64_t)w - 1;
  if (j > (int64_t)h - 1) j = (int64_t)h - 1;
  return (uint64_t)j * w + (uint64_t)i;
}
IZPI_DEV V3 image_at(const double* texels, uint64_t off, uint32_t fmt, uint64_t k) {
  if (fmt == TEXF_GRAY) {
    const double g = texels[off + k];
    return mk(g, g, g);
  }
  const double* px = texels + off + k * 4;
  const double2 rg = *reinterpret_cast<const double2*>(px);
  return mk(rg.x, rg.y, px[2]);
}
IZPI_DEV V3 tex_rgb(const DevScene& sc, int32_t id, double u, double v, bool st = false) {
  const izpi_texture t = tex_rec(sc, st, id);
  if (t.kind == IZPI_TEX_IMAGE) return image_rgb(sc.texels, t.texel_offset, t.width, t.height, t.pad0, u, v);
  return mk(t.value[0], t.value[1], t.value[2]);
}
IZPI_DEV V3 slot_rgb(const DevScene& sc, const TexSlot& s, double u, double v, bool st = false) {
  const uint32_t fmt = s.hf >> 30;
  if (fmt <= TEXF_GRAY) return image_rgb(sc.texels, s.off, s.w, s.hf & 0x3FFFFFFFu, fmt, u, v);
  return tex_rgb(sc, (int32_t)s.off, u, v, st);
}
IZPI_DEV bool slot_set(const TexSlot& s) { return (s.hf >> 30) != TEXF_NONE; }
IZPI_DEV V3 slot_rgb_k(const DevScene& sc, const TexSlot& s, double u, double v, bool st, uint32_t w0, uint32_t h0, uint64_t k0) {
  const uint32_t fmt = s.hf >> 30, h = s.hf & 0x3FFFFFFFu;
  if (fmt <= TEXF_GRAY) {
    uint64_t k = k0;
    if (s.w != w0 || h != h0) k = image_index(s.w, h, u, v);
    return image_at(sc.texels, s.off, fmt, k);
  }
  return slot_rgb(sc, s, u, v, st);
}
IZPI_DEV MatTex* mt_lds() { return (MatTex*)(lds_arena() + lds_off::MT); }
IZPI_DEV TexSlot mat_slot(const DevScene& sc, bool staged, uint32_t m, int k) {
  if (staged) return lds_ld(&mt_lds()[m].s[k]);
  return sc.mat_tex[m].s[k];
}
template <bool L = false>
IZPI_DEV uint32_t sorted_interval(const double* wl, uint32_t n, double w) {
  uint32_t lo = 1, hi = n - 1;
  while (lo < hi) {
    const uint32_t mid = (lo + hi) >> 1;
    if (tld<L>(wl + mid) >= w) hi = mid; else lo = mid + 1;
  }
  return lo - 1;
}

IZPI_DEV double spectral_image_value(double r, double g, double b, double wl) {
  double sv = 0;
// ... 964 lines not shown
  Shade shade, shade_staged;
  Tail tail32, tail64;
  Shade start;
  void (*refill)(DevScene, ShadeParams, WaveParams, const uint32_t*);
  uint32_t sampler, rec_doubles;
  int matset;
  bool fwd;
  char name[24];
};
template <int SAMPLER, bool FWD>
const ShadeKernels* shade_kernels(int matset);

struct SampleRange {
  uint32_t begin, end;
  bool keep;
};
struct ResolveParams {
  uint32_t num_pixels, done, width, height, tile_w, tile_h, sampler, out_layout;
  uint32_t form;
  double exposure;
  const uint32_t* tiles;
  const double* running;
  double* out;
};
void launch_resolve(hipStream_t st, const ResolveParams& rp);
struct NoiseParams {
  uint32_t num_pixels, done, width, height, tile_w, tile_h, sampler, out_layout;
  double threshold, floor;
  const uint32_t* tiles;
  const double* running;
  const double* moments;
  double* out;
  double* block_sums;
  unsigned long long* block_counts;
};
void launch_noise_resolve(hipStream_t st, const NoiseParams& np);
void launch_noise_stats(hipStream_t st, const NoiseParams& np);
static_assert(sizeof(RayOD) == izpi_internal::plan_size::RAY && sizeof(PathHot) == izpi_internal::plan_size::PATH_HOT &&
                  sizeof(PathCold) == izpi_internal::plan_size::PATH_COLD && sizeof(double2) == izpi_internal::plan_size::HIT,
              "render_plan.h: entry records");
static_assert(SMP_D == izpi_internal::plan_size::SMP_D && POOL_SHARDS == izpi_internal::plan_size::POOL_SHARDS,
              "render_plan.h: per-sample results, pool rings");
static_assert(RecLayout<IZPI_SAMPLER_COLOUR, MATSET_FULL>::D == izpi_internal::plan_size::REC_COLOUR &&
                  RecLayout<IZPI_SAMPLER_COLOUR, MATSET_CONST>::D == izpi_internal::plan_size::REC_COMPACT &&
                  RecLayout<IZPI_SAMPLER_SPECTRAL, MATSET_FULL>::D == izpi_internal::plan_size::REC_SPECTRAL,
              "render_plan.h: record strides");
struct DevBufs {
  std::vector<void*> p;
  template <typename T>
  hipError_t alloc(T** out, size_t count) {
    *out = nullptr;
    const hipError_t e = hipMalloc((void**)out, count * sizeof(T));
    if (e == hipSuccess) p.push_back(*out);
    return e;
  }
  ~DevBufs() {
    for (void* q : p) (void)hipFree(q);
  }
};

struct izpi_ctx {
  int device = 0;
  std::string err;
  hipStream_t stream = nullptr;
  hipEvent_t ev0 = nullptr, ev1 = nullptr, ev2 = nullptr;
  int num_cus = 0;
  bool have_scene = false;
  uint32_t num_textures = 0;
  uint32_t num_materials = 0;
  uint32_t num_spd = 0;
  izpi_internal::PlanCache plans[2];
  const GTriVerts* d_triverts = nullptr;
  DevScene sc{};
  uint32_t stack_needed = 0;
  uint32_t num_prims = 0;
  std::vector<void*> scene_allocs;
  size_t scene_bytes = 0;
  double* d_samples = nullptr; size_t samples_cap = 0;
  double* d_recs = nullptr; size_t recs_cap = 0;
  double* d_pool = nullptr; size_t pool_cap = 0;
  uint32_t* d_ring = nullptr; size_t ring_cap = 0;
  unsigned long long* d_pool_ctr = nullptr;
  double* d_running = nullptr; size_t running_cap = 0;
  double* d_out = nullptr; size_t out_cap = 0;
  uint32_t* d_tiles = nullptr; size_t tiles_cap = 0;
  uint32_t* d_utiles = nullptr; size_t utiles_cap = 0;
  double* d_bg = nullptr; size_t bg_cap = 0;
  uint32_t* d_misc = nullptr;
  unsigned long long* d_counters = nullptr;
  unsigned long long* d_cpart = nullptr; size_t cpart_cap = 0;
  unsigned long long* d_finq = nullptr; size_t finq_cap = 0;
  char* d_state = nullptr; size_t state_cap = 0;
  int32_t* d_spill = nullptr; size_t spill_cap = 0;
  double* d_post = nullptr; size_t post_cap = 0;
  double* d_share = nullptr; size_t share_cap = 0;
  double* d_gather = nullptr; size_t gather_cap = 0;
  double* d_denoise = nullptr; size_t denoise_cap = 0;
  double* d_moments = nullptr; size_t moments_cap = 0;
  double* d_noisepart = nullptr; size_t noisepart_cap = 0;
  uint32_t* h_count = nullptr;
  hipEvent_t ev3 = nullptr;
  hipEvent_t evb[3 * IZPI_PASS_BATCH] = {};
  ncclComm_t comm = nullptr;
  volatile uint32_t* stall_word = nullptr;
  uint32_t* stall_host = nullptr;
  uint32_t comm_rank = 0, comm_size = 1;
  int32_t* d_status = nullptr;
  int fault_inject = 0;
  izpi_render_stats last{};
  bool mat_ok_rgb = false, mat_ok_spectral = false;
  bool basic_materials = false;
  uint32_t matset = 0;
  bool const_albedo = false;
  bool any_uv = false;
  const ShadeKernels* kernels[2][2] = {};
  uint32_t pool_grow = 0;
  uint32_t dev_share = 1;
  std::atomic<uint64_t> prog_done{0}, prog_total{0};
  struct Session {
    bool open = false;
    bool broken = false;
    izpi_render_req req{};
    izpi_render_tuning tuning{};
    std::vector<uint32_t> tiles;
    std::vector<double> bg_wl, bg_val;
    uint32_t step_spp = 0, done = 0;
    bool noise = false;
    std::vector<uint32_t> run_tiles;
    uint32_t tile_w = 0, tile_h = 0, num_pixels = 0;
    izpi_render_stats cum{};
  } session;
};

inline uint32_t* misc(izpi_ctx* ctx, int k) { return ctx->d_misc + (size_t)k * MISC_STRIDE; }

template <typename K>
inline int resident_blocks(izpi_ctx* ctx, K kernel, int* blocks, int threads = 256, size_t dyn_lds = 0) {
  int per_cu = 0;
  if (dyn_lds) HIP_TRY(hipFuncSetAttribute((const void*)kernel, hipFuncAttributeMaxDynamicSharedMemorySize, (int)dyn_lds));
  HIP_TRY(hipOccupancyMaxActiveBlocksPerMultiprocessor(&per_cu, kernel, threads, dyn_lds));
  if (per_cu < 1) per_cu = 1;
  *blocks = per_cu * ctx->num_cus;
  return IZPI_OK;
}

constexpr int TRACE_RING = 16, TRACE_WPE = 5;
struct Tracer {
  bool p2 = true;
  bool tri = false;
  bool lds_bvh = false;
  bool ray_lds = false;
  bool qnodes = false;
  bool a32 = false;
  uint32_t prim_w = 32, tchunk = 512, refill_min = 24;
  int blocks = 0;
  size_t spill_bytes = 0;
};

const izpi_render_tuning kDefaultTuning{};

int make_tracer(izpi_ctx* ctx, const izpi_render_tuning& tu, bool need_uv, Tracer* t);
void launch_trace(izpi_ctx* ctx, const DevScene& sc, const Tracer& t, const WaveParams& wp, hipStream_t st, int32_t* spill);
int trace_ring(const Tracer& t);
struct RunInput { uint32_t num_pixels, chunk, pool_blocks; SampleRange range; };
struct RunTimes { float trace_ms = 0, shade_ms = 0, tail_ms = 0; uint32_t launches = 0; };
const ShadeKernels* shade_instance(uint32_t matset, bool const_basic, uint32_t sampler, bool fwd);
int run_wavefront(izpi_ctx* ctx, const izpi_render_req* req, const DevScene& sc, const Tracer& tr, const ShadeKernels& k,
                  ShadeParams& sp, WaveParams& wp, AccumParams& ap, const RunInput& in, RunTimes* out);
int prepare_wavefront(izpi_ctx* ctx, const ShadeKernels& k);
int prepare_accumulate(izpi_ctx* ctx);
void launch_accumulate(hipStream_t st, const AccumParams& ap, double* moments = nullptr);
inline double* session_moments(const izpi_ctx* ctx, const SampleRange& r) {
  return r.keep && ctx->session.noise ? ctx->d_moments : nullptr;
}
struct PreviewParams {
  WaveBuf buf;
  double2* tminmax;
  const GTriVerts* verts;
  double ink[3];
  uint32_t slots;
};
int run_preview(izpi_ctx* ctx, const izpi_render_req* req, const DevScene& sc, const Tracer& tr, ShadeParams& sp,
                const PreviewParams& pp, AccumParams& ap, const RunInput& in, RunTimes* out);
int prepare_preview(izpi_ctx* ctx);
inline bool preview_sampler(uint32_t s) {
  return s == IZPI_SAMPLER_NORMAL || s == IZPI_SAMPLER_ALBEDO || s == IZPI_SAMPLER_WIREFRAME;
}
inline double diag_clock_ms() {
  return std::chrono::duration<double, std::milli>(std::chrono::steady_clock::now().time_since_epoch()).count();
}
```

### izpi_amd/csrc/scene_pack.cpp

```cpp
#include "scene_pack.h"

#include <string.h>
#include <algorithm>
#include <cmath>

namespace izpi_internal {

using namespace izd;

bool stack_bound(const izpi_bvh4_node* nodes, size_t n, uint32_t* bound) {
  std::vector<uint32_t> best(n, 0);
  for (size_t k = n; k-- > 0;) {
    const izpi_bvh4_node& nd = nodes[k];
    if (nd.prim_count[0] > 0) continue;
    uint32_t valid = 0, deepest = 0;
    for (int i = 0; i < 4; i++) {
      if (nd.child[i] < 0) continue;
      valid++;
      if ((uint32_t)nd.child[i] <= k) return false;
      deepest = std::max(deepest, best[(size_t)nd.child[i]]);
    }
    best[k] = (valid ? valid - 1 : 0) + deepest;
  }
  *bound = n ? best[0] : 0;
  return true;
}

namespace {

int fail(std::string* err, int rc, const char* what) {
  *err = what;
  return rc;
}

int split_bvh(const izpi_scene_desc* d, PackedScene* out, std::vector<int32_t>& ref, std::string* err) {
  ref.assign(d->num_nodes, 0);
  uint32_t n_inner = 0;
  for (uint32_t k = 0; k < d->num_nodes; k++) {
    const izpi_bvh4_node& n = d->nodes[k];
    if (n.prim_count[0] > 0) {
      for (int i = 1; i < 4; i++)
        if (n.child[i] != -1) return fail(err, IZPI_ERR_INVALID, "leaf node with more than one slot");
      const int32_t st = n.child[0], cnt = n.prim_count[0];
      if (st < 0 || (uint64_t)st + (uint64_t)cnt > d->num_prims) return fail(err, IZPI_ERR_INVALID, "leaf primitive range out of bounds");
      if (cnt > 7 || st >= (1 << 27)) return fail(err, IZPI_ERR_UNSUPPORTED, "leaf too large for the leaf-ref encoding");
      ref[k] = make_leaf_ref(st, cnt);
    } else {
      for (int i = 0; i < 4; i++)
        if (n.prim_count[i] != 0) return fail(err, IZPI_ERR_INVALID, "inner node with a primitive slot");
      ref[k] = (int32_t)n_inner++;
    }
  }
  out->num_inner = n_inner;
  out->root = d->num_nodes ? ref[0] : -1;
  out->inner.assign(std::max<uint32_t>(1, n_inner), GInner{});
  out->leaves.assign(std::max<uint32_t>(1, d->num_prims), GLeaf{});
  out->leaf_shortcut = 1;
  for (uint32_t k = 0; k < d->num_nodes; k++) {
    const izpi_bvh4_node& n = d->nodes[k];
    if (ref[k] <= -2) {
      GLeaf& L = out->leaves[(size_t)leaf_start(ref[k])];
      L.mn[0] = n.min_x[0]; L.mn[1] = n.min_y[0]; L.mn[2] = n.min_z[0];
      L.mx[0] = n.max_x[0]; L.mx[1] = n.max_y[0]; L.mx[2] = n.max_z[0];
      L.start = n.child[0]; L.count = n.prim_count[0];
    } else {
      GInner& g = out->inner[(size_t)ref[k]];
      memcpy(g.mnx, n.min_x, 16); memcpy(g.mny, n.min_y, 16); memcpy(g.mnz, n.min_z, 16);
      memcpy(g.mxx, n.max_x, 16); memcpy(g.mxy, n.max_y, 16); memcpy(g.mxz, n.max_z, 16);
      for (int i = 0; i < 4; i++) {
        int32_t c = n.child[i];
        if (c != -1 && (c < 0 || (uint32_t)c >= d->num_nodes)) return fail(err, IZPI_ERR_INVALID, "child index out of bounds");
        g.child[i] = c == -1 ? -1 : ref[(size_t)c];
        g.pad[i] = 0;
        if (c >= 0 && ref[(size_t)c] <= -2) {
          const izpi_bvh4_node& lnode = d->nodes[(size_t)c];
          const float pb[6] = {n.min_x[i], n.min_y[i], n.min_z[i], n.max_x[i], n.max_y[i], n.max_z[i]};
          const float lb[6] = {lnode.min_x[0], lnode.min_y[0], lnode.min_z[0], lnode.max_x[0], lnode.max_y[0], lnode.max_z[0]};
          if (memcmp(pb, lb, sizeof(pb)) != 0) out->leaf_shortcut = 0;
        }
      }
    }
  }
  return IZPI_OK;
}

bool quantize_node(GInner& g, GInnerQ& q) {
  memset(&q, 0, sizeof(q));
  float* mn[3] = {g.mnx, g.mny, g.mnz};
  float* mx[3] = {g.mxx, g.mxy, g.mxz};
  for (int i = 0; i < 4; i++) q.child[i] = g.child[i];
  for (int a = 0; a < 3; a++) {
    float lo = 0.0f, hi = 0.0f;
    bool any = false;
    for (int i = 0; i < 4; i++) {
      if (g.child[i] == -1) continue;
      if (!std::isfinite(mn[a][i]) || !std::isfinite(mx[a][i])) return false;
      lo = any ? std::min(lo, mn[a][i]) : mn[a][i];
      hi = any ? std::max(hi, mx[a][i]) : mx[a][i];
      any = true;
    }
    const double ext = (double)hi - (double)lo;
    int e = -126;
    if (ext > 0) e = std::max(-126, (int)std::ceil(std::log2(ext / 255.0)));
    uint32_t qlo[4] = {0, 0, 0, 0}, qhi[4] = {0, 0, 0, 0};
    for (;; e++) {
      if (e > 127) return false;
      const float sc = std::ldexp(1.0f, e);
      bool ok = true;
      for (int i = 0; i < 4 && ok; i++) {
        if (g.child[i] == -1) continue;
        double fl = std::floor(((double)mn[a][i] - (double)lo) / (double)sc);
        int ql = (int)std::min(255.0, std::max(0.0, fl));
        while (ql > 0 && qdecode(lo, (uint32_t)ql, sc) > mn[a][i]) ql--;
        double fh = std::ceil(((double)mx[a][i] - (double)lo) / (double)sc);
        int qh = (int)std::max((double)ql, std::min(256.0, fh));
        while (qh <= 255 && qdecode(lo, (uint32_t)qh, sc) < mx[a][i]) qh++;
        if (qh > 255) ok = false;
        qlo[i] = (uint32_t)ql; qhi[i] = (uint32_t)qh;
      }
      if (ok) break;
    }
    const float sc = std::ldexp(1.0f, e);
    q.org[a] = lo;
    q.ex |= (uint32_t)(e + 127) << (8 * a);
    for (int i = 0; i < 4; i++) {
      q.q[a] |= qlo[i] << (8 * i);
      q.q[3 + a] |= qhi[i] << (8 * i);
      if (g.child[i] == -1) continue;
      mn[a][i] = qdecode(lo, qlo[i], sc);
      mx[a][i] = qdecode(lo, qhi[i], sc);
    }
  }
  return true;
}

void quantize_bvh(const izpi_scene_desc* d, PackedScene* out) {
  const uint32_t n_inner = out->num_inner;
  out->quantized = 0;
  if (!(d->abi_version >= 3 && (d->flags & IZPI_SCENE_QUANTIZED_BVH) && n_inner > 0)) return;
  std::vector<GInner> dec(out->inner);
  out->innerq.resize(n_inner);
  bool quantized = true;
  for (uint32_t k = 0; k < n_inner && quantized; k++) quantized = quantize_node(dec[k], out->innerq[k]);
  if (!quantized) {
    out->innerq.clear();
    return;
  }
  out->inner.swap(dec);
  for (uint32_t k = 0; k < n_inner; k++) {
    const GInner& g = out->inner[k];
    for (int i = 0; i < 4; i++) {
      if (!ref_is_leaf(g.child[i])) continue;
      GLeaf& L = out->leaves[(size_t)leaf_start(g.child[i])];
      L.mn[0] = g.mnx[i]; L.mn[1] = g.mny[i]; L.mn[2] = g.mnz[i];
      L.mx[0] = g.mxx[i]; L.mx[1] = g.mxy[i]; L.mx[2] = g.mxz[i];
    }
  }
  out->leaf_shortcut = 1;
  out->quantized = 1;
}

int pack_prims(const izpi_scene_desc* d, PackedScene* out, std::string* err) {
  const uint32_t nt = d->num_tris, ns = d->num_spheres;
  const bool tex = d->num_prims && (d->tri_uv || d->tri_tangent || d->tri_bitangent);
  out->prims.assign(d->num_prims, GPrim{});
  out->shade.assign(d->num_prims, GShade{});
  out->triverts.assign(std::max<uint32_t>(1, d->num_prims), GTriVerts{});
  out->tritex.assign(tex ? d->num_prims : 0, GTriTex{});
  for (uint32_t k = 0; k < d->num_prims; k++) {
    const uint32_t r = d->prim_ref[k], kind = IZPI_PRIM_KIND(r);
    const size_t idx = IZPI_PRIM_INDEX(r);
    GPrim& g = out->prims[k];
    g.kind = kind; g.index = (uint32_t)idx;
    GShade& gs = out->shade[k];
    gs.ref = r;
    if (kind == IZPI_PRIM_TRIANGLE) {
      if (idx >= nt) return fail(err, IZPI_ERR_INVALID, "triangle ref out of range");
      memcpy(gs.n, d->tri_normal + 3 * idx, 24);
      gs.mk = d->tri_mat[idx];
      memcpy(g.a, d->tri_v0 + 3 * idx, 24); memcpy(g.a + 3, d->tri_e1 + 3 * idx, 24);
      memcpy(g.a + 6, d->tri_e2 + 3 * idx, 24);
      memcpy(out->triverts[k].v1, d->tri_v1 + 3 * idx, 24);
      memcpy(out->triverts[k].v2, d->tri_v2 + 3 * idx, 24);
      if (tex && d->tri_uv) memcpy(out->tritex[k].uv, d->tri_uv + 6 * idx, 48);
      if (tex && d->tri_tangent) memcpy(out->tritex[k].tg, d->tri_tangent + 3 * idx, 24);
      if (tex && d->tri_bitangent) memcpy(out->tritex[k].bt, d->tri_bitangent + 3 * idx, 24);
    } else {
      if (idx >= ns) return fail(err, IZPI_ERR_INVALID, "sphere ref out of range");
      gs.mk = d->sph_mat[idx];
      memcpy(g.a, d->sph_center0 + 3 * idx, 24); memcpy(g.a + 3, d->sph_center1 + 3 * idx, 24);
      g.a[6] = d->sph_radius[idx]; g.a[7] = d->sph_time[2 * idx]; g.a[8] = d->sph_time[2 * idx + 1];
    }
  }
  return IZPI_OK;
}

int pack_lights(const izpi_scene_desc* d, PackedScene* out, std::string* err) {
  out->lights.assign(d->num_lights, GLight{});
  for (uint32_t i = 0; i < d->num_lights; i++) {
// ... 213 lines not shown
```

### izpi_amd/csrc/scene_pack.h

```cpp
#pragma once
#include <stddef.h>
#include <stdint.h>
#include <string>
#include <vector>

#include "scene_records.h"

namespace izpi_internal {

struct Double4 { double x, y, z, w; };

struct PackedScene {
  std::vector<izd::GInner> inner;
  std::vector<izd::GInnerQ> innerq;
  std::vector<izd::GLeaf> leaves;
  std::vector<izd::GPrim> prims;
  std::vector<izd::GShade> shade;
  std::vector<izd::GTriVerts> triverts;
  std::vector<izd::GTriTex> tritex;
  std::vector<izd::GLight> lights;
  std::vector<Double4> mat_const;
  std::vector<izd::MatTex> mat_tex;
  std::vector<izpi_texture> textures;
  std::vector<double> texels;
  int32_t root = -1;
  uint32_t num_inner = 0, leaf_shortcut = 1, quantized = 0, nan_free_bounds = 1, time_free = 1, no_pathlen = 1, tri_only = 1;
  uint32_t stack_needed = 0;
  bool mat_ok_rgb = true, mat_ok_spectral = true;
  bool basic_materials = true;
  uint32_t matset = 0;
  bool const_albedo = true;
  bool any_uv = false;
};

int pack_scene(const izpi_scene_desc* d, PackedScene* out, std::string* err);

struct TraceLayout { uint64_t innerq_at, leaves_at, bytes; };
inline TraceLayout trace_layout(uint64_t n_inner, uint64_t n_innerq, uint64_t n_leaves) {
  TraceLayout t;
  t.innerq_at = n_inner * sizeof(izd::GInner);
  t.leaves_at = t.innerq_at + n_innerq * sizeof(izd::GInnerQ);
  t.bytes = t.leaves_at + n_leaves * sizeof(izd::GLeaf);
  return t;
}
inline bool trace_addr32(uint64_t n_inner, uint64_t n_innerq, uint64_t n_leaves, uint64_t n_prims) {
  const uint64_t lim = 1ull << 32;
  return trace_layout(n_inner, n_innerq, n_leaves).bytes <= lim && n_prims * sizeof(izd::GPrim) <= lim;
}

bool stack_bound(const izpi_bvh4_node* nodes, size_t n, uint32_t* bound);

}
```

### izpi_amd/csrc/trace.hip

```cpp
#include "izpi_kern.h"

constexpr uint32_t BVH_LDS_BYTES = 4096;
__device__ __forceinline__ bool lane_of(uint64_t mask) { return __builtin_amdgcn_inverse_ballot_w64(mask); }
__device__ __forceinline__ uint32_t lanes_below(uint64_t mask) {
  return __builtin_amdgcn_mbcnt_hi((uint32_t)(mask >> 32), __builtin_amdgcn_mbcnt_lo((uint32_t)mask, 0u));
}
template <int S, int WPE, bool DIST, bool TRI, bool LB, bool RL, bool Q, bool A32>
__global__ void __launch_bounds__(256) __attribute__((amdgpu_waves_per_eu(WPE))) k_trace2(const DevScene sc, const WaveParams wp, unsigned long long* counters,
                                                uint32_t* err, int32_t* spill, uint32_t spill_stride, uint32_t prim_w,
                                                uint32_t tchunk, uint32_t refill_min) {
  static_assert((S & (S - 1)) == 0, "ring size must be a power of two");
  static_assert(!LB || DIST, "the LDS-resident BVH instance runs the distributed leaf tests");
  static_assert(!RL || (DIST && (TRI || LB)), "the LDS-resident ray instances: triangle-only global BVH, or the BVH in LDS");
  static_assert(!Q || !LB, "the quantised nodes are read from global memory");
  static_assert(!A32 || !LB, "the 32-bit offsets address records in global memory");
  constexpr bool UVL = !RL, UVS = RL && LB, DUV = !RL || LB;
  typedef float v4f __attribute__((ext_vector_type(4)));
  typedef double v2d __attribute__((ext_vector_type(2)));
  typedef const __attribute__((address_space(3))) v4f LF4;
  typedef const __attribute__((address_space(3))) v2d LD2;
  __shared__ float4 bvh_lds[LB ? BVH_LDS_BYTES / 16 : 1];
  LF4* const l_inner = (LF4*)bvh_lds;
  LF4* const l_leaves = l_inner + (size_t)8 * (LB ? sc.num_inner : 0);
  LD2* const l_prims = (LD2*)(l_leaves + (size_t)2 * (LB ? sc.num_prims : 0));
  if constexpr (LB) {
    const uint32_t ni = 8 * sc.num_inner, nl = 2 * sc.num_prims, np5 = 5 * sc.num_prims;
    for (uint32_t t = threadIdx.x; t < ni + nl + np5; t += 256)
      bvh_lds[t] = t < ni ? reinterpret_cast<const float4*>(sc.inner)[t]
                          : (t < ni + nl ? reinterpret_cast<const float4*>(sc.leaves)[t - ni]
                                         : reinterpret_cast<const float4*>(sc.prims)[t - ni - nl]);
    __syncthreads();
  }
  __shared__ int32_t lds_stack[S * 256];
  __shared__ uint32_t dist_owner[DIST ? 260 : 1];
  __shared__ double dist_t[DIST ? 260 : 1], dist_u[DIST && DUV ? 260 : 1], dist_v[DIST && DUV ? 260 : 1];
  __shared__ double2 lds_uv[UVL ? 256 : 1];
  __shared__ double2 ray_lds[RL ? 3 * 256 : 1];
  const uint32_t wbase = threadIdx.x & ~63u;
  constexpr uint32_t NODE_BYTES = Q ? sizeof(GInnerQ) : sizeof(GInner);
  const char* const nbase = Q ? reinterpret_cast<const char*>(sc.innerq) : reinterpret_cast<const char*>(sc.inner);
  const char* const pbase = reinterpret_cast<const char*>(sc.prims);
  const uint32_t leaf_off0 = A32 ? (uint32_t)(reinterpret_cast<const char*>(sc.leaves) - nbase) : 0u;
  int32_t* stk = lds_stack + threadIdx.x;
  int32_t* gsp = spill + blockIdx.x * 256 + threadIdx.x;
  const uint32_t lane = threadIdx.x & 63;
  const uint32_t n = *wp.in_count;
  if (wp.pool_ctr && blockIdx.x == 0) pool_publish(wp.pool_ctr);
  if (wp.out_count && blockIdx.x == 0 && threadIdx.x == 0) *wp.out_count = 0;
  if (wp.out_park && blockIdx.x == 0 && threadIdx.x == 0) *wp.out_park = 0;
  const bool read_kind = wp.read_kind != 0 || (wp.in_park && *wp.in_park != 0);
  const uint32_t nwaves = gridDim.x * 4u;
  const uint32_t chunk = min(tchunk, max(16u, (n + nwaves - 1u) / nwaves));
  const uint32_t first = chunk;
  if ((uint64_t)(blockIdx.x * 4u + (threadIdx.x >> 6)) * first >= n) return;
  uint64_t c_rays = 0, c_nodes = 0, c_tri = 0, c_sph = 0;
  uint64_t c_nstep = 0, c_pstep = 0, c_short = 0;
  bool busy = false, in_prim = false;
  bool exhausted = false;
  uint32_t qi = 0;
  uint32_t lkind = RAY_MAIN;
  double tmax = 0;
  float ix = 0, iy = 0, iz = 0, ox = 0, oy = 0, oz = 0;
  int32_t cur = -1, pk = 0, pend = 0;
  int32_t lref = 0;
  int sp = -1, low = 0;
  int clean_from = 0;
  int32_t bprim = -1;
  bool fast = false;
  uint64_t m_slow = ~0ull;
  bool any_spill = false;
#ifdef IZPI_SHADOW
  uint64_t c_spill_st = 0, c_spill_ld = 0;
  uint32_t sh_acc = 0;
#endif
  uint32_t c_pos = __builtin_amdgcn_readfirstlane((blockIdx.x * 4u + (threadIdx.x >> 6)) * first);
  uint32_t c_end = c_pos + first < n ? c_pos + first : n;
#ifdef IZPI_TRACE_CLOCKS
  uint64_t k_refill = 0, k_node = 0, k_prim = 0, k_adv = 0, k0 = 0, k1 = 0;
#define IZPI_CLK(v) (v) = __builtin_readcyclecounter()
#else
#define IZPI_CLK(v) (void)0
#endif
#ifdef IZPI_STEP_MARKS
#define IZPI_MARK(name) asm volatile("; IZPI_MARK " name)
#else
#define IZPI_MARK(name) (void)0
#endif
#ifdef IZPI_TRACE_ICOUNT
  uint32_t ic_iter = 0, ic_idle = 0, ic_dequeue = 0, ic_refill = 0, ic_twin = 0, ic_spill = 0, ic_readback = 0, ic_pop = 0, ic_finish = 0;
#define IZPI_IC(v) (v)++
#else
#define IZPI_IC(v) (void)0
#endif
  for (;;) {
    IZPI_CLK(k0);
    IZPI_MARK("head");
    IZPI_IC(ic_iter);
    const uint64_t idle = __builtin_amdgcn_ballot_w64(sp < 0);
    uint64_t idle_now = idle;
    if (idle != 0) {
      IZPI_MARK("idle");
      IZPI_IC(ic_idle);
      const uint32_t nidle = (uint32_t)__popcll(idle);
      if (!exhausted && (nidle >= refill_min || idle == ~0ull) && c_pos >= c_end) {
        IZPI_MARK("dequeue");
        IZPI_IC(ic_dequeue);
        uint32_t b = 0;
        if (lane == 0) b = atomicAdd(wp.trace_next, chunk);
        b = __builtin_amdgcn_readfirstlane(b) + nwaves * first;
        if (b >= n) exhausted = true;
        c_pos = b;
        c_end = b + chunk < n ? b + chunk : n;
      }
      if (!exhausted && (nidle >= refill_min || idle == ~0ull) && c_pos < c_end) {
        IZPI_MARK("refill");
        IZPI_IC(ic_refill);
        const uint32_t take = nidle < c_end - c_pos ? nidle : c_end - c_pos;
        const uint32_t base = c_pos;
        c_pos += take;
        bool main_ray = false;
        const uint32_t rank = lanes_below(idle);
        const uint32_t my = base + rank;
        if (!busy && rank < take) {
          const uint32_t k = read_kind ? sld(wp.in.kind + my) : (uint32_t)RAY_MAIN;
          RayOD r;
          if constexpr (RL) {
            r = sld(wp.in.ray + my);
            const double2* rp = reinterpret_cast<const double2*>(&r);
            const double2 r0 = rp[0], r1 = rp[1], r2 = rp[2];
            ray_lds[3 * threadIdx.x] = r0; ray_lds[3 * threadIdx.x + 1] = r1; ray_lds[3 * threadIdx.x + 2] = r2;
          } else {
            r = wp.in.ray[my];
          }
          if (!(k & (RAY_PARKED | RAY_DEAD)) && (uint64_t)__double_as_longlong(r.o[0]) != DEAD_BITS) {
            qi = my;
            lkind = k;
            tmax = ray_tmax(wp.in, my, k);
            main_ray = kind_of(k) == RAY_MAIN;
            ix = (float)(1.0 / r.d[0]); iy = (float)(1.0 / r.d[1]); iz = (float)(1.0 / r.d[2]);
            ox = (float)r.o[0]; oy = (float)r.o[1]; oz = (float)r.o[2];
            fast = sc.nan_free_bounds && ray_fast_ok(ox, oy, oz, ix, iy, iz);
            cur = sc.root;
            busy = cur != -1;
            sp = busy ? 0 : -1; low = 0; clean_from = 0;
            in_prim = false;
            bprim = -1;
            if (!busy) {
              if ((UVL || UVS) && wp.hit_uv) {
                double2* rec = wp.in.hit + ((size_t)my << 1);
                sst(rec, hit_pack(0.0, -1)); sst(rec + 1, make_double2(0.0, 0.0));
              } else {
                sst(wp.in.hit + my, hit_pack(0.0, -1));
              }
            }
          }
        }
        c_rays += (uint64_t)__popcll(__ballot(main_ray));
        m_slow = __ballot(!fast);
        idle_now = __builtin_amdgcn_ballot_w64(sp < 0);
        __builtin_amdgcn_s_waitcnt(0x0F70);
      } else if (exhausted && idle == ~0ull) {
        break;
      }
    }
    IZPI_MARK("pick");
    const uint64_t m_prim = DIST ? __builtin_amdgcn_ballot_w64(lref < 0) : __builtin_amdgcn_ballot_w64(pk < pend);
    const uint64_t m_node = ~(m_prim | idle_now);
    if ((m_prim | m_node) == 0) continue;
    const uint32_t n_prim = (uint32_t)__popcll(m_prim), n_node = (uint32_t)__popcll(m_node);
    bool advance = false;
    bool leaf_next = false;
    int32_t next = -1;
#ifdef IZPI_TRACE_CLOCKS
    IZPI_CLK(k1); k_refill += k1 - k0; k0 = k1;
    const bool clk_prim = n_prim * prim_w >= n_node * 16u;
#endif
    if (n_prim * prim_w >= n_node * 16u) {
      if constexpr (DIST) {
        IZPI_MARK("prim");
        const uint32_t cnt = lref < 0 ? (uint32_t)leaf_count(lref) : 0u;
        pk = leaf_start(lref);
        const uint32_t base = lanes_below(__ballot(cnt & 1u)) + 2u * lanes_below(__ballot(cnt & 2u)) +
                              4u * lanes_below(__ballot(cnt & 4u));
        const uint64_t ms = m_prim & __builtin_amdgcn_ballot_w64(base + cnt <= 64);
        const bool served = lane_of(ms);
        const int last = 63 - __clzll((long long)ms);
        const uint32_t total = (uint32_t)__builtin_amdgcn_readlane((int)(base + cnt), last);
        {
          const uint32_t e = ((uint32_t)pk << 6) | lane;
          uint32_t* dq = dist_owner + wbase + base;
          if (served) dq[0] = e;
          if (served && cnt > 1) dq[1] = e + 64u;
          if (served && cnt > 2) dq[2] = e + 128u;
          if (served && cnt > 3) dq[3] = e + 192u;
        }
        __builtin_amdgcn_wave_barrier();
        const uint32_t ent = lane < total ? dist_owner[wbase + lane] : lane;
        const uint32_t ow = ent & 63u;
        const uint32_t oqi = (uint32_t)__shfl((int)qi, (int)ow);
        const uint32_t okind = (uint32_t)__shfl((int)lkind, (int)ow);
        if (lane < total) {
          const int32_t pi = (int32_t)(ent >> 6);
          double2 r0, r1, r2;
          if constexpr (RL) {
            const uint32_t ro = 3 * (wbase + ow);
            r0 = ray_lds[ro]; r1 = ray_lds[ro + 1]; r2 = ray_lds[ro + 2];
          } else {
            const double2* rp = reinterpret_cast<const double2*>(wp.in.ray + oqi);
            r0 = rp[0]; r1 = rp[1]; r2 = rp[2];
          }
          const double otmin = ray_tmin(wp.in, oqi, okind);
          double2 p0, p1, p2, p3, p4;
          if constexpr (LB) {
            LD2* pp = l_prims + (size_t)5 * pi;
            const v2d a0 = pp[0], a1 = pp[1], a2 = pp[2], a3 = pp[3], a4 = pp[4];
            p0 = make_double2(a0.x, a0.y); p1 = make_double2(a1.x, a1.y); p2 = make_double2(a2.x, a2.y);
            p3 = make_double2(a3.x, a3.y); p4 = make_double2(a4.x, a4.y);
          } else {
            const double2* pp = A32 ? reinterpret_cast<const double2*>(pbase + (uint32_t)pi * (uint32_t)sizeof(GPrim))
                                    : reinterpret_cast<const double2*>(sc.prims + pi);
            p0 = pp[0]; p1 = pp[1]; p2 = pp[2]; p3 = pp[3]; p4 = pp[4];
#ifdef IZPI_SHADOW
            if (IZPI_SHADOW & 4) {
              const uint4* sq = reinterpret_cast<const uint4*>(sc.sh_prims + pi);
              const uint4 s0 = sq[0], s1 = sq[1], s2 = sq[2], s3 = sq[3], s4 = sq[4];
              sh_acc ^= s0.x ^ s1.y ^ s2.z ^ s3.w ^ s4.x;
            }
#endif
          }
          const double pa[9] = {p0.x, p0.y, p1.x, p1.y, p2.x, p2.y, p3.x, p3.y, p4.x};
          double t = 0, u = 0, v = 0;
          const V3 o = mk(r0.x, r0.y, r1.x), d = mk(r1.y, r2.x, r2.y);
          uint32_t flags;
          if (TRI || (uint32_t)__double2loint(p4.y) == IZPI_PRIM_TRIANGLE) {
            flags = tri_intersect_no_tmax(pa, o, d, otmin, t, u, v) ? 1u : 0u;
          } else {
            const double time = (RL && LB) || sc.time_free ? pa[7] : (wp.in.time ? wp.in.time[oqi] : 0.0);
            flags = 2u;
            if (sph_roots(sph_center(pa, time), pa[6], o, d, t, u))
              flags |= 1u | (t > otmin ? 4u : 0u) | (u > otmin ? 8u : 0u);
          }
          dist_t[wbase + lane] = t;
          if constexpr (DUV) { dist_u[wbase + lane] = u; dist_v[wbase + lane] = v; }
          dist_owner[wbase + lane] = flags;
        }
        const uint32_t n_sph_tests = TRI ? 0u : (uint32_t)__popcll(__ballot(lane < total && (dist_owner[wbase + lane] & 2u)));
        __builtin_amdgcn_wave_barrier();
        if (served && (TRI || n_sph_tests == 0)) {
          const uint32_t j0 = wbase + base;
          uint32_t f[4];
          double tt[4];
#pragma unroll
          for (uint32_t i = 0; i < 4; i++) { f[i] = dist_owner[j0 + i]; tt[i] = dist_t[j0 + i]; }
          int32_t acc = -1;
#pragma unroll
          for (uint32_t i = 0; i < 4; i++)
            if (i < cnt && (f[i] & 1u) && !(tt[i] > tmax)) { tmax = tt[i]; acc = (int32_t)i; }
          if (acc >= 0) {
            if constexpr (UVL) lds_uv[threadIdx.x] = make_double2(dist_u[j0 + acc], dist_v[j0 + acc]);
            if constexpr (UVS)
              if (wp.hit_uv) sst(wp.in.hit + ((size_t)qi << 1) + 1, make_double2(dist_u[j0 + acc], dist_v[j0 + acc]));
            bprim = pk + acc;
            clean_from = sp;
          }
          lref = 0;
          in_prim = false;
          advance = true;
        } else if (!TRI && served) {
          int32_t acc = -1;
          double acc_u = 0, acc_v = 0;
          for (uint32_t i = 0; i < cnt; i++) {
            const uint32_t j = wbase + base + i;
            const uint32_t f = dist_owner[j];
            if (!(f & 1u)) continue;
            if (!(f & 2u)) {
              const double t = dist_t[j];
              if (!(t > tmax)) { tmax = t; acc = (int32_t)j; acc_u = dist_u[j]; acc_v = dist_v[j]; bprim = pk + (int32_t)i; }
            } else {
              const double ta = dist_t[j], tb = dist_u[j];
              if (ta < tmax && (f & 4u)) { tmax = ta; acc = (int32_t)j; acc_u = 0.0; acc_v = 0.0; bprim = pk + (int32_t)i; }
              else if (tb < tmax && (f & 8u)) { tmax = tb; acc = (int32_t)j; acc_u = 1.0; acc_v = 0.0; bprim = pk + (int32_t)i; }
            }
          }
          if (acc >= 0) {
            if constexpr (UVS) {
              if (wp.hit_uv) sst(wp.in.hit + ((size_t)qi << 1) + 1, make_double2(acc_u, acc_v));
            } else {
              lds_uv[threadIdx.x] = make_double2(acc_u, acc_v);
            }
            clean_from = sp;
          }
          lref = 0;
          in_prim = false;
          advance = true;
        }
        __builtin_amdgcn_wave_barrier();
        c_tri += total - n_sph_tests;
        c_sph += n_sph_tests;
        c_pstep++;
      } else {
      bool is_tri = false;
      if (busy && in_prim) {
        const double2* rp = reinterpret_cast<const double2*>(wp.in.ray + qi);
        const double2 r0 = rp[0], r1 = rp[1], r2 = rp[2];
        const V3 o = mk(r0.x, r0.y, r1.x), d = mk(r1.y, r2.x, r2.y);
        const double tmin = ray_tmin(wp.in, qi, lkind);
        const double2* pp = A32 ? reinterpret_cast<const double2*>(pbase + (uint32_t)pk * (uint32_t)sizeof(GPrim))
                                : reinterpret_cast<const double2*>(sc.prims + pk);
        const double2 p0 = pp[0], p1 = pp[1], p2 = pp[2], p3 = pp[3], p4 = pp[4];
        const double pa[9] = {p0.x, p0.y, p1.x, p1.y, p2.x, p2.y, p3.x, p3.y, p4.x};
        is_tri = TRI || (uint32_t)__double2loint(p4.y) == IZPI_PRIM_TRIANGLE;
        if (is_tri) {
          double t, u, v;
          if (tri_intersect(pa, o, d, tmin, tmax, t, u, v)) {
            tmax = t; bprim = pk; lds_uv[threadIdx.x] = make_double2(u, v); clean_from = sp;
          }
        } else if (!TRI) {
          const double time = wp.in.time ? wp.in.time[qi] : 0.0;
          double t; int root;
          if (sph_intersect(pa, o, d, time, tmin, tmax, t, root)) {
            tmax = t; bprim = pk; lds_uv[threadIdx.x] = make_double2((double)root, 0.0); clean_from = sp;
          }
        }
        pk++;
        if (pk == pend) { in_prim = false; advance = true; }
      }
      const uint32_t n_tri = (uint32_t)__popcll(__ballot(is_tri));
      c_tri += n_tri;
      c_sph += n_prim - n_tri;
      c_pstep++;
      }
    } else {
      IZPI_MARK("node");
      c_nodes += n_node;
      c_nstep++;
      const bool wave_fast = (m_node & m_slow) == 0;
#ifdef IZPI_TRACE_ICOUNT
      if (!wave_fast) ic_twin++;
#endif
      if ((m_node & __builtin_amdgcn_ballot_w64(sp + 3 - low > S)) != 0) {
        IZPI_MARK("spill");
        any_spill = true;
        IZPI_IC(ic_spill);
        if (busy && !in_prim) {
          while (sp + 3 - low > S) {
            gsp[(size_t)low * spill_stride] = stk[(low & (S - 1)) * 256];
            low++;
#ifdef IZPI_SHADOW
            c_spill_st++;
#endif
          }
        }
      }
      IZPI_MARK("node_loads");
      if (busy && !in_prim) {
        const float tm = (float)tmax;
        const bool is_leaf = ref_is_leaf(cur);
        float4 q0, q1, mnz_, mxx_, mxy_, mxz_;
        int4 ch_;
        const float4 *lp = nullptr, *np = nullptr;
        if constexpr (!LB && A32) {
          const uint32_t noff = is_leaf ? 0u : (uint32_t)cur * NODE_BYTES;
          const uint32_t loff = is_leaf ? leaf_off0 + (uint32_t)leaf_start(cur) * (uint32_t)sizeof(GLeaf) : noff;
          lp = reinterpret_cast<const float4*>(nbase + loff);
          np = reinterpret_cast<const float4*>(nbase + noff);
        } else if constexpr (!LB) {
          lp = reinterpret_cast<const float4*>(is_leaf ? (const void*)(sc.leaves + leaf_start(cur))
                                                       : Q ? (const void*)(sc.innerq + cur) : (const void*)(sc.inner + cur));
          np = is_leaf ? reinterpret_cast<const float4*>(nbase) : lp;
        }
        if constexpr (LB) {
          LF4* llp = is_leaf ? l_leaves + (size_t)2 * leaf_start(cur) : l_inner + (size_t)8 * cur;
          LF4* lnp = is_leaf ? l_inner : llp;
          const v4f a0 = llp[0], a1 = llp[1], a2 = lnp[2], a3 = lnp[3], a4 = lnp[4], a5 = lnp[5], c = lnp[6];
          q0 = make_float4(a0.x, a0.y, a0.z, a0.w); q1 = make_float4(a1.x, a1.y, a1.z, a1.w);
          mnz_ = make_float4(a2.x, a2.y, a2.z, a2.w); mxx_ = make_float4(a3.x, a3.y, a3.z, a3.w);
          mxy_ = make_float4(a4.x, a4.y, a4.z, a4.w); mxz_ = make_float4(a5.x, a5.y, a5.z, a5.w);
          ch_ = make_int4(__float_as_int(c.x), __float_as_int(c.y), __float_as_int(c.z), __float_as_int(c.w));
        } else if constexpr (Q) {
          q0 = lp[0]; q1 = lp[1];
          const float4 c2 = np[2], c3 = np[3];
          const uint32_t ex = __float_as_uint(q0.w);
          const float sx = __uint_as_float((ex & 0xFFu) << 23), sy = __uint_as_float(((ex >> 8) & 0xFFu) << 23),
                      sz = __uint_as_float(((ex >> 16) & 0xFFu) << 23);
          auto dec4 = [](float w, float o, float sc_) {
            const uint32_t b = __float_as_uint(w);
            return make_float4(__builtin_fmaf((float)(b & 0xFFu), sc_, o), __builtin_fmaf((float)((b >> 8) & 0xFFu), sc_, o),
                               __builtin_fmaf((float)((b >> 16) & 0xFFu), sc_, o), __builtin_fmaf((float)(b >> 24), sc_, o));
          };
          const float4 dmnx = dec4(q1.x, q0.x, sx), dmny = dec4(q1.y, q0.y, sy), dmnz = dec4(q1.z, q0.z, sz);
          const float4 dmxx = dec4(q1.w, q0.x, sx), dmxy = dec4(c2.x, q0.y, sy), dmxz = dec4(c2.y, q0.z, sz);
          const float4 l0 = q0, l1 = q1;
          q0 = is_leaf ? l0 : dmnx;
          q1 = is_leaf ? l1 : make_float4(dmny.x, dmny.y, dmny.z, dmny.w);
          mnz_ = dmnz; mxx_ = dmxx; mxy_ = dmxy; mxz_ = dmxz;
          ch_ = make_int4(__float_as_int(c2.z), __float_as_int(c2.w), __float_as_int(c3.x), __float_as_int(c3.y));
        } else {
          q0 = lp[0]; q1 = lp[1];
          mnz_ = np[2]; mxx_ = np[3]; mxy_ = np[4]; mxz_ = np[5];
          ch_ = *reinterpret_cast<const int4*>(np + 6);
#ifdef IZPI_SHADOW
          if ((IZPI_SHADOW & 1) && !is_leaf) {
            const uint4* sq = reinterpret_cast<const uint4*>(sc.sh_inner + cur);
            const uint4 s0 = sq[0], s1 = sq[1], s2 = sq[2], s3 = sq[3], s4 = sq[4], s5 = sq[5], s6 = sq[6];
            sh_acc ^= s0.x ^ s1.y ^ s2.z ^ s3.w ^ s4.x ^ s5.y ^ s6.z;
          }
          if ((IZPI_SHADOW & 2) && is_leaf) {
            const uint4* sq = reinterpret_cast<const uint4*>(sc.sh_leaves + leaf_start(cur));
            const uint4 s0 = sq[0], s1 = sq[1];
            sh_acc ^= s0.x ^ s1.y;
          }
#endif
        }
        const float4 mnx = q0;
        const float4 mny = make_float4(is_leaf ? q0.y : q1.x, q1.y, q1.z, q1.w);
        const float4 mnz = make_float4(is_leaf ? q0.z : mnz_.x, mnz_.y, mnz_.z, mnz_.w);
        const float4 mxx = make_float4(is_leaf ? q0.w : mxx_.x, mxx_.y, mxx_.z, mxx_.w);
        const float4 mxy = make_float4(is_leaf ? q1.x : mxy_.x, mxy_.y, mxy_.z, mxy_.w);
        const float4 mxz = make_float4(is_leaf ? q1.y : mxz_.x, mxz_.y, mxz_.z, mxz_.w);
        const int4 ch = make_int4(is_leaf ? cur : ch_.x, ch_.y, ch_.z, ch_.w);
        uint64_t hit[4];
        if (wave_fast) {
          IZPI_MARK("slab_fast");
          slab4_fast(mnx, mny, mnz, mxx, mxy, mxz, ox, oy, oz, ix, iy, iz, tm, hit);
        } else {
          IZPI_MARK("slab_twin");
          const float amnx[4] = {mnx.x, mnx.y, mnx.z, mnx.w}, amny[4] = {mny.x, mny.y, mny.z, mny.w},
                      amnz[4] = {mnz.x, mnz.y, mnz.z, mnz.w}, amxx[4] = {mxx.x, mxx.y, mxx.z, mxx.w},
                      amxy[4] = {mxy.x, mxy.y, mxy.z, mxy.w}, amxz[4] = {mxz.x, mxz.y, mxz.z, mxz.w};
#pragma unroll
          for (int i = 0; i < 4; i++)
            hit[i] = __builtin_amdgcn_ballot_w64(slab(amnx[i], amny[i], amnz[i], amxx[i], amxy[i], amxz[i], ox, oy, oz, ix, iy, iz, tm));
        }
        IZPI_MARK("node_tail");
        const uint64_t m_inner = __builtin_amdgcn_ballot_w64(cur >= -1);
        const uint64_t b0 = hit[0] & __builtin_amdgcn_ballot_w64(ch.x != -1),
                       b1 = hit[1] & m_inner & __builtin_amdgcn_ballot_w64(ch.y != -1),
                       b2 = hit[2] & m_inner & __builtin_amdgcn_ballot_w64(ch.z != -1),
                       b3 = hit[3] & m_inner & __builtin_amdgcn_ballot_w64(ch.w != -1);
        next = lane_of(b3) ? ch.w : -1;
        next = lane_of(b2) ? ch.z : next;
        next = lane_of(b1) ? ch.y : next;
        next = lane_of(b0) ? ch.x : next;
        const bool enter = ref_is_leaf(next) && (is_leaf || sc.leaf_shortcut);
        leaf_next = enter && !is_leaf;
        in_prim = enter;
        if constexpr (DIST) {
          lref = enter ? next : lref;
        } else {
          pk = enter ? leaf_start(next) : pk;
          pend = enter ? leaf_start(next) + leaf_count(next) : pend;
        }
        next = enter ? -1 : next;
        const uint64_t r1 = b0 & b1, r2 = (b0 | b1) & b2, r3 = (b0 | b1 | b2) & b3;
        const int np_ = (int)lane_of(r1) + (int)lane_of(r2) + (int)lane_of(r3);
        const int32_t e0z = lane_of(r2) ? ch.z : ch.w;
        const int32_t e0 = lane_of(r1) ? ch.y : e0z;
        const int32_t e1 = lane_of(r1 & r2) ? ch.z : ch.w;
        stk[(sp & (S - 1)) * 256] = e0;
        stk[((sp + 1) & (S - 1)) * 256] = e1;
        stk[((sp + 2) & (S - 1)) * 256] = ch.w;
        if (sp + np_ > 64) atomicOr(err, 1u);
        sp += np_;
        advance = !enter;
      }
    }
#ifdef IZPI_TRACE_CLOCKS
    IZPI_CLK(k1); if (clk_prim) k_prim += k1 - k0; else k_node += k1 - k0; k0 = k1;
#endif
    {
      IZPI_MARK("advance");
      const bool do_pop = advance && next == -1 && sp > 0;
      const bool do_fin = advance && next == -1 && sp == 0;
      const int spn = sp - 1;
      int32_t top = *(volatile __attribute__((address_space(3))) int32_t*)&lds_stack[threadIdx.x + (spn & (S - 1)) * 256];
#ifdef IZPI_TRACE_ICOUNT
      if (__ballot(do_pop) != 0) ic_pop++;
      if (__ballot(do_fin) != 0) ic_finish++;
#endif
      if (any_spill && __ballot(do_pop && spn < low) != 0) {
        IZPI_MARK("readback");
        IZPI_IC(ic_readback);
        if (do_pop && spn < low) {
          top = gsp[(size_t)spn * spill_stride];
          low = spn;
#ifdef IZPI_SHADOW
          c_spill_ld++;
#endif
        }
        __builtin_amdgcn_s_waitcnt(0x0F70);
      }
      IZPI_MARK("advance_tail");
      cur = (advance && next != -1) ? next : (do_pop ? top : cur);
      sp = (advance && next == -1) ? spn : sp;
      const bool lf = do_pop && ref_is_leaf(top) && spn >= clean_from && sc.leaf_shortcut;
      in_prim = in_prim || lf;
      leaf_next = leaf_next || lf;
      if constexpr (DIST) {
        lref = lf ? top : lref;
      } else {
        pk = lf ? leaf_start(top) : pk;
        pend = lf ? leaf_start(top) + leaf_count(top) : pend;
      }
      clean_from = (do_pop && spn < clean_from) ? spn : clean_from;
      if (do_fin) {
        IZPI_MARK("finish");
        const double2 uv = (UVL && bprim >= 0) ? lds_uv[threadIdx.x] : make_double2(0.0, 0.0);
        if ((UVL || UVS) && wp.hit_uv) {
          double2* rec = wp.in.hit + ((size_t)qi << 1);
          sst(rec, hit_pack(bprim >= 0 ? tmax : 0.0, bprim));
          if (!UVS || bprim < 0) sst(rec + 1, uv);
        } else {
          sst(wp.in.hit + qi, hit_pack(bprim >= 0 ? tmax : 0.0, bprim));
        }
        busy = false;
      }
    }
    IZPI_MARK("advance_end");
    const uint64_t n_short = (uint64_t)__popcll(__builtin_amdgcn_ballot_w64(leaf_next));
    c_nodes += n_short;
    c_short += n_short;
#ifdef IZPI_TRACE_CLOCKS
    IZPI_CLK(k1); k_adv += k1 - k0;
#endif
  }
#ifdef IZPI_TRACE_CLOCKS
  if (lane == 0) {
    atomicAdd(counters + CNT_CLK_REFILL, (unsigned long long)k_refill);
    atomicAdd(counters + CNT_CLK_NODE, (unsigned long long)k_node);
    atomicAdd(counters + CNT_CLK_PRIM, (unsigned long long)k_prim);
    atomicAdd(counters + CNT_CLK_ADV, (unsigned long long)k_adv);
  }
#endif
#ifdef IZPI_SHADOW
  {
    if (c_spill_st) atomicAdd(counters + CNT_CLK_REFILL, (unsigned long long)c_spill_st);
    if (c_spill_ld) atomicAdd(counters + CNT_CLK_NODE, (unsigned long long)c_spill_ld);
    if (sh_acc == 0x9E3779B9u) atomicOr(err, 0u);
  }
#endif
#ifdef IZPI_TRACE_ICOUNT
  if (lane == 0) {
    count_add(wp.cpart, counters, CNT_IC_ITER, ic_iter);
    count_add(wp.cpart, counters, CNT_IC_IDLE, ic_idle);
    count_add(wp.cpart, counters, CNT_IC_DEQUEUE, ic_dequeue);
    count_add(wp.cpart, counters, CNT_IC_REFILL, ic_refill);
    count_add(wp.cpart, counters, CNT_IC_TWIN, ic_twin);
    count_add(wp.cpart, counters, CNT_IC_SPILL, ic_spill);
    count_add(wp.cpart, counters, CNT_IC_READBACK, ic_readback);
    count_add(wp.cpart, counters, CNT_IC_POP, ic_pop);
    count_add(wp.cpart, counters, CNT_IC_FINISH, ic_finish);
    count_add(wp.cpart, counters, CNT_IC_WAVES, 1);
  }
#endif
  if (lane == 0) {
    count_add(wp.cpart, counters, CNT_RAYS, c_rays);
    count_add(wp.cpart, counters, CNT_NODES, c_nodes);
    count_add(wp.cpart, counters, CNT_TRI, c_tri);
    count_add(wp.cpart, counters, CNT_SPH, c_sph);
    count_add(wp.cpart, counters, CNT_NSTEP, c_nstep);
    count_add(wp.cpart, counters, CNT_PSTEP, c_pstep);
    count_add(wp.cpart, counters, CNT_SHORT, c_short);
  }
}


#define IZPI_T2_LIST(X)                                                                                           \
  X(true, false, false, false, false) X(true, true, false, false, false) X(false, false, false, false, false)        \
  X(false, true, false, false, false) X(true, false, true, false, false) X(true, true, true, false, false)           \
  X(true, true, false, true, false) X(true, false, true, true, false) X(true, true, true, true, false)               \
  X(true, false, false, false, true) X(true, true, false, false, true) X(true, true, false, true, true)
constexpr int ring_of(bool lb, bool rl) { return lb && rl ? 8 : TRACE_RING; }
int trace_ring(const Tracer& t) { return ring_of(t.lds_bvh, t.ray_lds); }

int make_tracer(izpi_ctx* ctx, const izpi_render_tuning& tu, bool need_uv, Tracer* t) {
  *t = Tracer();
  if (tu.flags & IZPI_TUNE_NO_DIST) t->p2 = false;
  if (ctx->num_prims >= (1u << 26)) t->p2 = false;
  t->tri = ctx->sc.tri_only != 0 && !(tu.flags & IZPI_TUNE_GENERAL_TRACE);
  t->lds_bvh = t->p2 && !(tu.flags & IZPI_TUNE_NO_LDS_BVH) &&
               (uint64_t)ctx->sc.num_inner * sizeof(GInner) + (uint64_t)ctx->sc.num_prims * (sizeof(GLeaf) + sizeof(GPrim)) <= BVH_LDS_BYTES;
  if (t->lds_bvh) {
    t->refill_min = 40;
    t->prim_w = 24;
  }
  t->ray_lds = t->p2 && ((t->tri && !t->lds_bvh && !need_uv) || (t->lds_bvh && (t->tri || ctx->sc.time_free))) &&
               !(tu.flags & IZPI_TUNE_NO_RAY_LDS);
  t->qnodes = ctx->sc.quantized && t->p2 && !t->lds_bvh && !(tu.flags & IZPI_TUNE_NO_QNODES);
  t->a32 = ctx->sc.addr32 != 0 && !(tu.flags & IZPI_TUNE_WIDE_ADDR);
  if (tu.prim_weight) t->prim_w = tu.prim_weight;
  if (tu.trace_chunk) t->tchunk = tu.trace_chunk;
  if (tu.refill_min) t->refill_min = std::min<uint32_t>(64, tu.refill_min);
  int rc = IZPI_ERR_INVALID;
  ctx->err = "no k_trace2 instance for this scene and tuning";
#define IZPI_T2_OCC(P, T, L, R, Q)                                                               \
  if (t->p2 == P && t->tri == T && t->lds_bvh == L && t->ray_lds == R && t->qnodes == Q) \
    rc = t->a32 ? resident_blocks(ctx, k_trace2<ring_of(L, R), TRACE_WPE, P, T, L, R, Q, !L>, &t->blocks)       \
                : resident_blocks(ctx, k_trace2<ring_of(L, R), TRACE_WPE, P, T, L, R, Q, false>, &t->blocks);
  IZPI_T2_LIST(IZPI_T2_OCC)
#undef IZPI_T2_OCC
  if (rc) return rc;
  t->spill_bytes = (size_t)t->blocks * 256 * 64 * sizeof(int32_t);
  return IZPI_OK;
}

void launch_trace(izpi_ctx* ctx, const DevScene& sc, const Tracer& t, const WaveParams& wp, hipStream_t st, int32_t* spill) {
  const dim3 g(t.blocks), b(256);
  const uint32_t stride = (uint32_t)t.blocks * 256;
#define IZPI_T2_LAUNCH(P, T, L, R, Q)                                                                          \
  if (t.p2 == P && t.tri == T && t.lds_bvh == L && t.ray_lds == R && t.qnodes == Q) {                          \
    if (t.a32)                                                                                                 \
      hipLaunchKernelGGL((k_trace2<ring_of(L, R), TRACE_WPE, P, T, L, R, Q, !L>), g, b, 0, st, sc, wp,           \
                         ctx->d_counters, misc(ctx, 1), spill, stride, t.prim_w, t.tchunk, t.refill_min);       \
    else                                                                                                       \
      hipLaunchKernelGGL((k_trace2<ring_of(L, R), TRACE_WPE, P, T, L, R, Q, false>), g, b, 0, st, sc, wp,        \
                         ctx->d_counters, misc(ctx, 1), spill, stride, t.prim_w, t.tchunk, t.refill_min);       \
    return;                                                                                                    \
  }
  IZPI_T2_LIST(IZPI_T2_LAUNCH)
#undef IZPI_T2_LAUNCH
}
```

Measured before the change: 2604.

## Specialize trace kernel for three-prim leaves and fixed tMin; rework lane state masks

```diff
diff --git a/include/izpi_gpu.h b/include/izpi_gpu.h
--- a/include/izpi_gpu.h
+++ b/include/izpi_gpu.h
@@ -87,7 +87,8 @@
   IZPI_TUNE_NO_PLACE_PICK = 512,
   IZPI_TUNE_NO_QNODES = 1024,
   IZPI_TUNE_NO_SHADE_STAGE = 2048,
-  IZPI_TUNE_WIDE_ADDR = 4096
+  IZPI_TUNE_WIDE_ADDR = 4096,
+  IZPI_TUNE_LEAF4 = 8192
 };
 
 typedef struct izpi_render_req {
diff --git a/izpi_amd/_native.py b/izpi_amd/_native.py
--- a/izpi_amd/_native.py
+++ b/izpi_amd/_native.py
@@ -97,6 +97,7 @@
 TUNE_NO_QNODES = 1024
 TUNE_NO_SHADE_STAGE = 2048
 TUNE_WIDE_ADDR = 4096
+TUNE_LEAF4 = 8192
 
 
 def tuning(**kw):
diff --git a/izpi_amd/csrc/izpi_dev.h b/izpi_amd/csrc/izpi_dev.h
--- a/izpi_amd/csrc/izpi_dev.h
+++ b/izpi_amd/csrc/izpi_dev.h
@@ -37,6 +37,7 @@
   uint32_t time_free;
   uint32_t quantized;
   uint32_t addr32;
+  uint32_t leaf_max;
 #ifdef IZPI_SHADOW
   const GInner* sh_inner;
   const GLeaf* sh_leaves;
diff --git a/izpi_amd/csrc/izpi_gpu.hip b/izpi_amd/csrc/izpi_gpu.hip
--- a/izpi_amd/csrc/izpi_gpu.hip
+++ b/izpi_amd/csrc/izpi_gpu.hip
@@ -594,8 +594,8 @@
   const double t_tiles = host_ms();
   if ((rc = make_tracer(ctx, tu, !ctx->sc.tri_only || ctx->any_uv, &tr))) return rc;
   if (pass_log)
-    fprintf(stderr, "IZPI_TRACE_INSTANCE dist=%d tri=%d lds_bvh=%d ray_lds=%d q=%d\nIZPI_TRACE_ADDR a32=%d ring=%d\n", (int)tr.p2, (int)tr.tri,
-            (int)tr.lds_bvh, (int)tr.ray_lds, (int)tr.qnodes, (int)(tr.a32 && !tr.lds_bvh), trace_ring(tr));
+    fprintf(stderr, "IZPI_TRACE_INSTANCE dist=%d tri=%d lds_bvh=%d ray_lds=%d q=%d\nIZPI_TRACE_ADDR a32=%d ring=%d\nIZPI_TRACE_LEAVES leaf_max=%u leaf3=%d tmin_fixed=%d\n", (int)tr.p2, (int)tr.tri,
+            (int)tr.lds_bvh, (int)tr.ray_lds, (int)tr.qnodes, (int)(tr.a32 && !tr.lds_bvh), trace_ring(tr), ctx->sc.leaf_max, (int)tr.leaf3, (int)(ctx->sc.no_pathlen != 0));
   const double t_tracer = host_ms();
   PlanCache& cache = ctx->plans[rs.preview];
   PlanInput in = plan_input(ctx, req, rs, tu, call.size_spp);
@@ -684,10 +684,10 @@
   fprintf(stderr, "IZPI_SHADOW spill_stores %llu spill_loads %llu (entries)\n", cnt[CNT_CLK_REFILL], cnt[CNT_CLK_NODE]);
 #endif
 #ifdef IZPI_TRACE_ICOUNT
-  fprintf(stderr, "IZPI_TRACE_ICOUNT {\"iterations\": %llu, \"idle\": %llu, \"dequeue\": %llu, \"refill\": %llu, \"prim\": %llu, \"node_fast\": %llu, "
-          "\"node_twin\": %llu, \"spill\": %llu, \"readback\": %llu, \"pop\": %llu, \"finish\": %llu, \"waves\": %llu}\n",
-          cnt[CNT_IC_ITER], cnt[CNT_IC_IDLE], cnt[CNT_IC_DEQUEUE], cnt[CNT_IC_REFILL], cnt[CNT_PSTEP], cnt[CNT_NSTEP] - cnt[CNT_IC_TWIN], cnt[CNT_IC_TWIN],
-          cnt[CNT_IC_SPILL], cnt[CNT_IC_READBACK], cnt[CNT_IC_POP], cnt[CNT_IC_FINISH], cnt[CNT_IC_WAVES]);
+  fprintf(stderr, "IZPI_TRACE_ICOUNT {\"iterations\": %llu, \"due\": %llu, \"dequeue\": %llu, \"refill\": %llu, \"prim\": %llu, \"node_fast\": %llu, "
+          "\"node_twin\": %llu, \"spill\": %llu, \"readback\": %llu, \"spilled\": %llu, \"pop\": %llu, \"finish\": %llu, \"waves\": %llu}\n",
+          cnt[CNT_IC_ITER], cnt[CNT_IC_DUE], cnt[CNT_IC_DEQUEUE], cnt[CNT_IC_REFILL], cnt[CNT_PSTEP], cnt[CNT_NSTEP] - cnt[CNT_IC_TWIN], cnt[CNT_IC_TWIN],
+          cnt[CNT_IC_SPILL], cnt[CNT_IC_READBACK], cnt[CNT_IC_SPILLED], cnt[CNT_IC_POP], cnt[CNT_IC_FINISH], cnt[CNT_IC_WAVES]);
 #endif
 #ifdef IZPI_TRACE_CLOCKS
   fprintf(stderr, "IZPI_TRACE_CLOCKS refill %llu node %llu prim %llu advance %llu (wave cycles)\n", cnt[CNT_CLK_REFILL],
@@ -1080,7 +1080,7 @@
   sc.spd_wl = dswl; sc.spd_val = dsv;
   sc.root = ps.root; sc.num_inner = ps.num_inner; sc.num_prims = d->num_prims; sc.num_lights = d->num_lights;
   sc.quantized = ps.quantized; sc.leaf_shortcut = ps.leaf_shortcut; sc.nan_free_bounds = ps.nan_free_bounds;
-  sc.tri_only = ps.tri_only; sc.time_free = ps.time_free; sc.no_pathlen = ps.no_pathlen;
+  sc.tri_only = ps.tri_only; sc.time_free = ps.time_free; sc.no_pathlen = ps.no_pathlen; sc.leaf_max = ps.leaf_max;
   sc.addr32 = trace_addr32(ps.inner.size(), ps.innerq.size(), ps.leaves.size(), ps.prims.size());
   sc.cam = d->camera;
   ctx->d_triverts = dtv;
diff --git a/izpi_amd/csrc/izpi_kern.h b/izpi_amd/csrc/izpi_kern.h
--- a/izpi_amd/csrc/izpi_kern.h
+++ b/izpi_amd/csrc/izpi_kern.h
@@ -64,7 +64,7 @@
 #ifdef IZPI_TRACE_ICOUNT
 enum { CNT_IC_ITER = CNT_CLK_REFILL, CNT_IC_DEQUEUE = CNT_CLK_NODE, CNT_IC_REFILL = CNT_CLK_PRIM, CNT_IC_TWIN = CNT_CLK_ADV,
        CNT_IC_SPILL = CNT_SCLK_ITEM, CNT_IC_READBACK = CNT_SCLK_REFILL, CNT_IC_POP = CNT_SCLK_PUSH, CNT_IC_FINISH = CNT_SCLK_MAT,
-       CNT_IC_WAVES = CNT_SCLK_FIN, CNT_IC_IDLE = CNT_SCLK_MIX };
+       CNT_IC_WAVES = CNT_SCLK_FIN, CNT_IC_DUE = CNT_SCLK_MIX, CNT_IC_SPILLED = CNT_SCLK_LPDF };
 #if defined(IZPI_TRACE_CLOCKS) || defined(IZPI_SHADE_CLOCKS) || defined(IZPI_SHADOW)
 #error "IZPI_TRACE_ICOUNT shares counter rows with the clock and shadow builds"
 #endif
@@ -1335,6 +1335,7 @@
   bool ray_lds = false;
   bool qnodes = false;
   bool a32 = false;
+  bool leaf3 = false;
   uint32_t prim_w = 32, tchunk = 512, refill_min = 24;
   int blocks = 0;
   size_t spill_bytes = 0;
diff --git a/izpi_amd/csrc/scene_pack.cpp b/izpi_amd/csrc/scene_pack.cpp
--- a/izpi_amd/csrc/scene_pack.cpp
+++ b/izpi_amd/csrc/scene_pack.cpp
@@ -45,6 +45,7 @@
       if (st < 0 || (uint64_t)st + (uint64_t)cnt > d->num_prims) return fail(err, IZPI_ERR_INVALID, "leaf primitive range out of bounds");
       if (cnt > 7 || st >= (1 << 27)) return fail(err, IZPI_ERR_UNSUPPORTED, "leaf too large for the leaf-ref encoding");
       ref[k] = make_leaf_ref(st, cnt);
+      out->leaf_max = std::max(out->leaf_max, (uint32_t)cnt);
     } else {
       for (int i = 0; i < 4; i++)
         if (n.prim_count[i] != 0) return fail(err, IZPI_ERR_INVALID, "inner node with a primitive slot");
diff --git a/izpi_amd/csrc/scene_pack.h b/izpi_amd/csrc/scene_pack.h
--- a/izpi_amd/csrc/scene_pack.h
+++ b/izpi_amd/csrc/scene_pack.h
@@ -26,6 +26,7 @@
   int32_t root = -1;
   uint32_t num_inner = 0, leaf_shortcut = 1, quantized = 0, nan_free_bounds = 1, time_free = 1, no_pathlen = 1, tri_only = 1;
   uint32_t stack_needed = 0;
+  uint32_t leaf_max = 0;
   bool mat_ok_rgb = true, mat_ok_spectral = true;
   bool basic_materials = true;
   uint32_t matset = 0;
diff --git a/izpi_amd/csrc/trace.hip b/izpi_amd/csrc/trace.hip
--- a/izpi_amd/csrc/trace.hip
+++ b/izpi_amd/csrc/trace.hip
@@ -5,7 +5,7 @@
 __device__ __forceinline__ uint32_t lanes_below(uint64_t mask) {
   return __builtin_amdgcn_mbcnt_hi((uint32_t)(mask >> 32), __builtin_amdgcn_mbcnt_lo((uint32_t)mask, 0u));
 }
-template <int S, int WPE, bool DIST, bool TRI, bool LB, bool RL, bool Q, bool A32>
+template <int S, int WPE, bool DIST, bool TRI, bool LB, bool RL, bool Q, bool A32, bool L3, bool FT>
 __global__ void __launch_bounds__(256) __attribute__((amdgpu_waves_per_eu(WPE))) k_trace2(const DevScene sc, const WaveParams wp, unsigned long long* counters,
                                                 uint32_t* err, int32_t* spill, uint32_t spill_stride, uint32_t prim_w,
                                                 uint32_t tchunk, uint32_t refill_min) {
@@ -14,6 +14,9 @@
   static_assert(!RL || (DIST && (TRI || LB)), "the LDS-resident ray instances: triangle-only global BVH, or the BVH in LDS");
   static_assert(!Q || !LB, "the quantised nodes are read from global memory");
   static_assert(!A32 || !LB, "the 32-bit offsets address records in global memory");
+  static_assert(!L3 || DIST, "the leaf size bound shapes the distributed primitive step");
+  static_assert(!FT || L3, "the fixed tMin is compiled for the three-primitive leaf instances");
+  constexpr uint32_t LEAF_MAX = L3 ? 3 : 4;
   constexpr bool UVL = !RL, UVS = RL && LB, DUV = !RL || LB;
   typedef float v4f __attribute__((ext_vector_type(4)));
   typedef double v2d __attribute__((ext_vector_type(2)));
@@ -55,7 +58,7 @@
   if ((uint64_t)(blockIdx.x * 4u + (threadIdx.x >> 6)) * first >= n) return;
   uint64_t c_rays = 0, c_nodes = 0, c_tri = 0, c_sph = 0;
   uint64_t c_nstep = 0, c_pstep = 0, c_short = 0;
-  bool busy = false, in_prim = false;
+  uint64_t m_scan = 0;
   bool exhausted = false;
   uint32_t qi = 0;
   uint32_t lkind = RAY_MAIN;
@@ -87,7 +90,7 @@
 #define IZPI_MARK(name) (void)0
 #endif
 #ifdef IZPI_TRACE_ICOUNT
-  uint32_t ic_iter = 0, ic_idle = 0, ic_dequeue = 0, ic_refill = 0, ic_twin = 0, ic_spill = 0, ic_readback = 0, ic_pop = 0, ic_finish = 0;
+  uint32_t ic_iter = 0, ic_due = 0, ic_spilled = 0, ic_dequeue = 0, ic_refill = 0, ic_twin = 0, ic_spill = 0, ic_readback = 0, ic_pop = 0, ic_finish = 0;
 #define IZPI_IC(v) (v)++
 #else
 #define IZPI_IC(v) (void)0
@@ -98,11 +101,12 @@
     IZPI_IC(ic_iter);
     const uint64_t idle = __builtin_amdgcn_ballot_w64(sp < 0);
     uint64_t idle_now = idle;
-    if (idle != 0) {
-      IZPI_MARK("idle");
-      IZPI_IC(ic_idle);
-      const uint32_t nidle = (uint32_t)__popcll(idle);
-      if (!exhausted && (nidle >= refill_min || idle == ~0ull) && c_pos >= c_end) {
+    if (exhausted && idle == ~0ull) break;
+    const uint32_t nidle = (uint32_t)__popcll(idle);
+    if (nidle >= refill_min && !exhausted) {
+      IZPI_MARK("due");
+      IZPI_IC(ic_due);
+      if (c_pos >= c_end) {
         IZPI_MARK("dequeue");
         IZPI_IC(ic_dequeue);
         uint32_t b = 0;
@@ -112,7 +116,7 @@
         c_pos = b;
         c_end = b + chunk < n ? b + chunk : n;
       }
-      if (!exhausted && (nidle >= refill_min || idle == ~0ull) && c_pos < c_end) {
+      if (!exhausted) {
         IZPI_MARK("refill");
         IZPI_IC(ic_refill);
         const uint32_t take = nidle < c_end - c_pos ? nidle : c_end - c_pos;
@@ -121,7 +125,7 @@
         bool main_ray = false;
         const uint32_t rank = lanes_below(idle);
         const uint32_t my = base + rank;
-        if (!busy && rank < take) {
+        if (lane_of(idle) && rank < take) {
           const uint32_t k = read_kind ? sld(wp.in.kind + my) : (uint32_t)RAY_MAIN;
           RayOD r;
           if constexpr (RL) {
@@ -141,11 +145,9 @@
             ox = (float)r.o[0]; oy = (float)r.o[1]; oz = (float)r.o[2];
             fast = sc.nan_free_bounds && ray_fast_ok(ox, oy, oz, ix, iy, iz);
             cur = sc.root;
-            busy = cur != -1;
-            sp = busy ? 0 : -1; low = 0; clean_from = 0;
-            in_prim = false;
+            sp = cur != -1 ? 0 : -1; low = 0; clean_from = 0;
             bprim = -1;
-            if (!busy) {
+            if (cur == -1) {
               if ((UVL || UVS) && wp.hit_uv) {
                 double2* rec = wp.in.hit + ((size_t)my << 1);
                 sst(rec, hit_pack(0.0, -1)); sst(rec + 1, make_double2(0.0, 0.0));
@@ -159,17 +161,20 @@
         m_slow = __ballot(!fast);
         idle_now = __builtin_amdgcn_ballot_w64(sp < 0);
         __builtin_amdgcn_s_waitcnt(0x0F70);
-      } else if (exhausted && idle == ~0ull) {
-        break;
       }
     }
     IZPI_MARK("pick");
     const uint64_t m_prim = DIST ? __builtin_amdgcn_ballot_w64(lref < 0) : __builtin_amdgcn_ballot_w64(pk < pend);
     const uint64_t m_node = ~(m_prim | idle_now);
+    {
+      const uint64_t n_short = (uint64_t)__popcll(m_prim & ~m_scan);
+      c_nodes += n_short;
+      c_short += n_short;
+      m_scan = m_prim;
+    }
     if ((m_prim | m_node) == 0) continue;
     const uint32_t n_prim = (uint32_t)__popcll(m_prim), n_node = (uint32_t)__popcll(m_node);
-    bool advance = false;
-    bool leaf_next = false;
+    uint64_t m_down = 0, m_up = 0;
     int32_t next = -1;
 #ifdef IZPI_TRACE_CLOCKS
     IZPI_CLK(k1); k_refill += k1 - k0; k0 = k1;
@@ -180,8 +185,8 @@
         IZPI_MARK("prim");
         const uint32_t cnt = lref < 0 ? (uint32_t)leaf_count(lref) : 0u;
         pk = leaf_start(lref);
-        const uint32_t base = lanes_below(__ballot(cnt & 1u)) + 2u * lanes_below(__ballot(cnt & 2u)) +
-                              4u * lanes_below(__ballot(cnt & 4u));
+        uint32_t base = lanes_below(__ballot(cnt & 1u)) + 2u * lanes_below(__ballot(cnt & 2u));
+        if constexpr (!L3) base += 4u * lanes_below(__ballot(cnt & 4u));
         const uint64_t ms = m_prim & __builtin_amdgcn_ballot_w64(base + cnt <= 64);
         const bool served = lane_of(ms);
         const int last = 63 - __clzll((long long)ms);
@@ -192,13 +197,15 @@
           if (served) dq[0] = e;
           if (served && cnt > 1) dq[1] = e + 64u;
           if (served && cnt > 2) dq[2] = e + 128u;
-          if (served && cnt > 3) dq[3] = e + 192u;
+          if constexpr (!L3)
+            if (served && cnt > 3) dq[3] = e + 192u;
         }
         __builtin_amdgcn_wave_barrier();
         const uint32_t ent = lane < total ? dist_owner[wbase + lane] : lane;
         const uint32_t ow = ent & 63u;
-        const uint32_t oqi = (uint32_t)__shfl((int)qi, (int)ow);
-        const uint32_t okind = (uint32_t)__shfl((int)lkind, (int)ow);
+        uint32_t oqi = 0, okind = (uint32_t)RAY_MAIN;
+        if constexpr (!RL || !FT) oqi = (uint32_t)__shfl((int)qi, (int)ow);
+        if constexpr (!FT) okind = (uint32_t)__shfl((int)lkind, (int)ow);
         if (lane < total) {
           const int32_t pi = (int32_t)(ent >> 6);
           double2 r0, r1, r2;
@@ -209,7 +216,7 @@
             const double2* rp = reinterpret_cast<const double2*>(wp.in.ray + oqi);
             r0 = rp[0]; r1 = rp[1]; r2 = rp[2];
           }
-          const double otmin = ray_tmin(wp.in, oqi, okind);
+          const double otmin = FT ? 0.001 : ray_tmin(wp.in, oqi, okind);
           double2 p0, p1, p2, p3, p4;
           if constexpr (LB) {
             LD2* pp = l_prims + (size_t)5 * pi;
@@ -248,13 +255,13 @@
         __builtin_amdgcn_wave_barrier();
         if (served && (TRI || n_sph_tests == 0)) {
           const uint32_t j0 = wbase + base;
-          uint32_t f[4];
-          double tt[4];
+          uint32_t f[LEAF_MAX];
+          double tt[LEAF_MAX];
 #pragma unroll
-          for (uint32_t i = 0; i < 4; i++) { f[i] = dist_owner[j0 + i]; tt[i] = dist_t[j0 + i]; }
+          for (uint32_t i = 0; i < LEAF_MAX; i++) { f[i] = dist_owner[j0 + i]; tt[i] = dist_t[j0 + i]; }
           int32_t acc = -1;
 #pragma unroll
-          for (uint32_t i = 0; i < 4; i++)
+          for (uint32_t i = 0; i < LEAF_MAX; i++)
             if (i < cnt && (f[i] & 1u) && !(tt[i] > tmax)) { tmax = tt[i]; acc = (int32_t)i; }
           if (acc >= 0) {
             if constexpr (UVL) lds_uv[threadIdx.x] = make_double2(dist_u[j0 + acc], dist_v[j0 + acc]);
@@ -264,8 +271,6 @@
             clean_from = sp;
           }
           lref = 0;
-          in_prim = false;
-          advance = true;
         } else if (!TRI && served) {
           int32_t acc = -1;
           double acc_u = 0, acc_v = 0;
@@ -291,16 +296,16 @@
             clean_from = sp;
           }
           lref = 0;
-          in_prim = false;
-          advance = true;
         }
         __builtin_amdgcn_wave_barrier();
+        m_scan = m_prim & ~ms;
+        m_up = ms;
         c_tri += total - n_sph_tests;
         c_sph += n_sph_tests;
         c_pstep++;
       } else {
       bool is_tri = false;
-      if (busy && in_prim) {
+      if (lane_of(m_prim)) {
         const double2* rp = reinterpret_cast<const double2*>(wp.in.ray + qi);
         const double2 r0 = rp[0], r1 = rp[1], r2 = rp[2];
         const V3 o = mk(r0.x, r0.y, r1.x), d = mk(r1.y, r2.x, r2.y);
@@ -323,8 +328,9 @@
           }
         }
         pk++;
-        if (pk == pend) { in_prim = false; advance = true; }
-      }
+      }
+      m_scan = __builtin_amdgcn_ballot_w64(pk < pend);
+      m_up = m_prim & ~m_scan;
       const uint32_t n_tri = (uint32_t)__popcll(__ballot(is_tri));
       c_tri += n_tri;
       c_sph += n_prim - n_tri;
@@ -342,7 +348,7 @@
         IZPI_MARK("spill");
         any_spill = true;
         IZPI_IC(ic_spill);
-        if (busy && !in_prim) {
+        if (lane_of(m_node)) {
           while (sp + 3 - low > S) {
             gsp[(size_t)low * spill_stride] = stk[(low & (S - 1)) * 256];
             low++;
@@ -353,7 +359,8 @@
         }
       }
       IZPI_MARK("node_loads");
-      if (busy && !in_prim) {
+      const uint64_t m_inner = __builtin_amdgcn_ballot_w64(cur >= -1);
+      if (lane_of(m_node)) {
         const float tm = (float)tmax;
         const bool is_leaf = ref_is_leaf(cur);
         float4 q0, q1, mnz_, mxx_, mxy_, mxz_;
@@ -433,7 +440,6 @@
             hit[i] = __builtin_amdgcn_ballot_w64(slab(amnx[i], amny[i], amnz[i], amxx[i], amxy[i], amxz[i], ox, oy, oz, ix, iy, iz, tm));
         }
         IZPI_MARK("node_tail");
-        const uint64_t m_inner = __builtin_amdgcn_ballot_w64(cur >= -1);
         const uint64_t b0 = hit[0] & __builtin_amdgcn_ballot_w64(ch.x != -1),
                        b1 = hit[1] & m_inner & __builtin_amdgcn_ballot_w64(ch.y != -1),
                        b2 = hit[2] & m_inner & __builtin_amdgcn_ballot_w64(ch.z != -1),
@@ -443,8 +449,6 @@
         next = lane_of(b1) ? ch.y : next;
         next = lane_of(b0) ? ch.x : next;
         const bool enter = ref_is_leaf(next) && (is_leaf || sc.leaf_shortcut);
-        leaf_next = enter && !is_leaf;
-        in_prim = enter;
         if constexpr (DIST) {
           lref = enter ? next : lref;
         } else {
@@ -460,42 +464,53 @@
         stk[(sp & (S - 1)) * 256] = e0;
         stk[((sp + 1) & (S - 1)) * 256] = e1;
         stk[((sp + 2) & (S - 1)) * 256] = ch.w;
-        if (sp + np_ > 64) atomicOr(err, 1u);
+        if (sp + np_ > 64) {
+          IZPI_MARK("overflow");
+          atomicOr(err, 1u);
+        }
         sp += np_;
-        advance = !enter;
-      }
+      }
+      const uint64_t m_after = DIST ? __builtin_amdgcn_ballot_w64(lref < 0) : __builtin_amdgcn_ballot_w64(pk < pend);
+      const uint64_t n_short = (uint64_t)__popcll(m_after & ~m_prim & m_inner);
+      c_nodes += n_short;
+      c_short += n_short;
+      m_scan = m_after;
+      m_down = __builtin_amdgcn_ballot_w64(next != -1);
+      m_up = m_node & ~(m_down | (m_after & ~m_prim));
     }
 #ifdef IZPI_TRACE_CLOCKS
     IZPI_CLK(k1); if (clk_prim) k_prim += k1 - k0; else k_node += k1 - k0; k0 = k1;
 #endif
     {
       IZPI_MARK("advance");
-      const bool do_pop = advance && next == -1 && sp > 0;
-      const bool do_fin = advance && next == -1 && sp == 0;
+      const uint64_t m_pop = m_up & __builtin_amdgcn_ballot_w64(sp > 0), m_fin = m_up & ~m_pop;
+      const bool do_pop = lane_of(m_pop), do_fin = lane_of(m_fin);
       const int spn = sp - 1;
       int32_t top = *(volatile __attribute__((address_space(3))) int32_t*)&lds_stack[threadIdx.x + (spn & (S - 1)) * 256];
 #ifdef IZPI_TRACE_ICOUNT
-      if (__ballot(do_pop) != 0) ic_pop++;
-      if (__ballot(do_fin) != 0) ic_finish++;
-#endif
-      if (any_spill && __ballot(do_pop && spn < low) != 0) {
-        IZPI_MARK("readback");
-        IZPI_IC(ic_readback);
-        if (do_pop && spn < low) {
-          top = gsp[(size_t)spn * spill_stride];
-          low = spn;
+      if (m_pop != 0) ic_pop++;
+      if (m_fin != 0) ic_finish++;
+#endif
+      if (any_spill) {
+        IZPI_MARK("spilled");
+        IZPI_IC(ic_spilled);
+        if (__ballot(do_pop && spn < low) != 0) {
+          IZPI_MARK("readback");
+          IZPI_IC(ic_readback);
+          if (do_pop && spn < low) {
+            top = gsp[(size_t)spn * spill_stride];
+            low = spn;
 #ifdef IZPI_SHADOW
-          c_spill_ld++;
-#endif
-        }
-        __builtin_amdgcn_s_waitcnt(0x0F70);
+            c_spill_ld++;
+#endif
+          }
+          __builtin_amdgcn_s_waitcnt(0x0F70);
+        }
       }
       IZPI_MARK("advance_tail");
-      cur = (advance && next != -1) ? next : (do_pop ? top : cur);
-      sp = (advance && next == -1) ? spn : sp;
+      cur = lane_of(m_down) ? next : (do_pop ? top : cur);
+      sp = lane_of(m_up) ? spn : sp;
       const bool lf = do_pop && ref_is_leaf(top) && spn >= clean_from && sc.leaf_shortcut;
-      in_prim = in_prim || lf;
-      leaf_next = leaf_next || lf;
       if constexpr (DIST) {
         lref = lf ? top : lref;
       } else {
@@ -513,13 +528,9 @@
         } else {
           sst(wp.in.hit + qi, hit_pack(bprim >= 0 ? tmax : 0.0, bprim));
         }
-        busy = false;
       }
     }
     IZPI_MARK("advance_end");
-    const uint64_t n_short = (uint64_t)__popcll(__builtin_amdgcn_ballot_w64(leaf_next));
-    c_nodes += n_short;
-    c_short += n_short;
 #ifdef IZPI_TRACE_CLOCKS
     IZPI_CLK(k1); k_adv += k1 - k0;
 #endif
@@ -542,7 +553,8 @@
 #ifdef IZPI_TRACE_ICOUNT
   if (lane == 0) {
     count_add(wp.cpart, counters, CNT_IC_ITER, ic_iter);
-    count_add(wp.cpart, counters, CNT_IC_IDLE, ic_idle);
+    count_add(wp.cpart, counters, CNT_IC_DUE, ic_due);
+    count_add(wp.cpart, counters, CNT_IC_SPILLED, ic_spilled);
     count_add(wp.cpart, counters, CNT_IC_DEQUEUE, ic_dequeue);
     count_add(wp.cpart, counters, CNT_IC_REFILL, ic_refill);
     count_add(wp.cpart, counters, CNT_IC_TWIN, ic_twin);
@@ -573,6 +585,26 @@
 constexpr int ring_of(bool lb, bool rl) { return lb && rl ? 8 : TRACE_RING; }
 int trace_ring(const Tracer& t) { return ring_of(t.lds_bvh, t.ray_lds); }
 
+typedef void (*TraceKernel)(const DevScene, const WaveParams, unsigned long long*, uint32_t*, int32_t*, uint32_t, uint32_t,
+                            uint32_t, uint32_t);
+template <bool P, bool T, bool L, bool R, bool Q>
+static TraceKernel trace_instance(bool a32, bool leaf3, bool tmin_fixed) {
+  constexpr int S = ring_of(L, R);
+  if (a32 && !L) {
+    if (leaf3 && P) return tmin_fixed ? k_trace2<S, TRACE_WPE, P, T, L, R, Q, !L, P, P> : k_trace2<S, TRACE_WPE, P, T, L, R, Q, !L, P, false>;
+    return k_trace2<S, TRACE_WPE, P, T, L, R, Q, !L, false, false>;
+  }
+  if (leaf3 && P) return tmin_fixed ? k_trace2<S, TRACE_WPE, P, T, L, R, Q, false, P, P> : k_trace2<S, TRACE_WPE, P, T, L, R, Q, false, P, false>;
+  return k_trace2<S, TRACE_WPE, P, T, L, R, Q, false, false, false>;
+}
+static TraceKernel trace_kernel(const Tracer& t, bool tmin_fixed) {
+#define IZPI_T2_PICK(P, T, L, R, Q) \
+  if (t.p2 == P && t.tri == T && t.lds_bvh == L && t.ray_lds == R && t.qnodes == Q) return trace_instance<P, T, L, R, Q>(t.a32, t.leaf3, tmin_fixed);
+  IZPI_T2_LIST(IZPI_T2_PICK)
+#undef IZPI_T2_PICK
+  return nullptr;
+}
+
 int make_tracer(izpi_ctx* ctx, const izpi_render_tuning& tu, bool need_uv, Tracer* t) {
   *t = Tracer();
   if (tu.flags & IZPI_TUNE_NO_DIST) t->p2 = false;
@@ -588,17 +620,16 @@
                !(tu.flags & IZPI_TUNE_NO_RAY_LDS);
   t->qnodes = ctx->sc.quantized && t->p2 && !t->lds_bvh && !(tu.flags & IZPI_TUNE_NO_QNODES);
   t->a32 = ctx->sc.addr32 != 0 && !(tu.flags & IZPI_TUNE_WIDE_ADDR);
+  t->leaf3 = t->p2 && ctx->sc.leaf_max <= 3 && !(tu.flags & IZPI_TUNE_LEAF4);
   if (tu.prim_weight) t->prim_w = tu.prim_weight;
   if (tu.trace_chunk) t->tchunk = tu.trace_chunk;
   if (tu.refill_min) t->refill_min = std::min<uint32_t>(64, tu.refill_min);
-  int rc = IZPI_ERR_INVALID;
-  ctx->err = "no k_trace2 instance for this scene and tuning";
-#define IZPI_T2_OCC(P, T, L, R, Q)                                                               \
-  if (t->p2 == P && t->tri == T && t->lds_bvh == L && t->ray_lds == R && t->qnodes == Q) \
-    rc = t->a32 ? resident_blocks(ctx, k_trace2<ring_of(L, R), TRACE_WPE, P, T, L, R, Q, !L>, &t->blocks)       \
-                : resident_blocks(ctx, k_trace2<ring_of(L, R), TRACE_WPE, P, T, L, R, Q, false>, &t->blocks);
-  IZPI_T2_LIST(IZPI_T2_OCC)
-#undef IZPI_T2_OCC
+  const TraceKernel k = trace_kernel(*t, false);
+  if (!k) {
+    ctx->err = "no k_trace2 instance for this scene and tuning";
+    return IZPI_ERR_INVALID;
+  }
+  const int rc = resident_blocks(ctx, k, &t->blocks);
   if (rc) return rc;
   t->spill_bytes = (size_t)t->blocks * 256 * 64 * sizeof(int32_t);
   return IZPI_OK;
@@ -607,16 +638,7 @@
 void launch_trace(izpi_ctx* ctx, const DevScene& sc, const Tracer& t, const WaveParams& wp, hipStream_t st, int32_t* spill) {
   const dim3 g(t.blocks), b(256);
   const uint32_t stride = (uint32_t)t.blocks * 256;
-#define IZPI_T2_LAUNCH(P, T, L, R, Q)                                                                          \
-  if (t.p2 == P && t.tri == T && t.lds_bvh == L && t.ray_lds == R && t.qnodes == Q) {                          \
-    if (t.a32)                                                                                                 \
-      hipLaunchKernelGGL((k_trace2<ring_of(L, R), TRACE_WPE, P, T, L, R, Q, !L>), g, b, 0, st, sc, wp,           \
-                         ctx->d_counters, misc(ctx, 1), spill, stride, t.prim_w, t.tchunk, t.refill_min);       \
-    else                                                                                                       \
-      hipLaunchKernelGGL((k_trace2<ring_of(L, R), TRACE_WPE, P, T, L, R, Q, false>), g, b, 0, st, sc, wp,        \
-                         ctx->d_counters, misc(ctx, 1), spill, stride, t.prim_w, t.tchunk, t.refill_min);       \
-    return;                                                                                                    \
-  }
-  IZPI_T2_LIST(IZPI_T2_LAUNCH)
-#undef IZPI_T2_LAUNCH
+  const bool tmin_fixed = sc.no_pathlen != 0 && wp.in.tminmax == nullptr;
+  hipLaunchKernelGGL(trace_kernel(t, tmin_fixed), g, b, 0, st, sc, wp, ctx->d_counters, misc(ctx, 1), spill, stride, t.prim_w, t.tchunk,
+                     t.refill_min);
 }
```

Result: faster. 2703, median of 6 (+3.8%).
